# opencv/opencv_contrib

Hardware: AMD Instinct MI355X
Metric: frame-pairs/sec dense TV-L1 flow @1080p (higher is better)
Workload: dtype f32; 1 GPU; DualTVL1 dense flow, 1920x1080 CV_32FC1, 64 pairs/GPU/step (BASELINE configs[1]; 64 pairs/GPU = the per-GPU share of ~; warps=5, nscales=5, semantics=CPU_REF, math=fast, lanes=2

## Files before the change

opencv_contrib_amd/csrc/mi_common.cpp:

```cpp
#include "mi_common.h"
#include <vector>
#include <cstdlib>
#include <cstring>
#include <cstdio>
#include <mutex>

namespace mi {
static Tuning g_tuning;
static std::once_flag g_tuning_once;
static int env_int(const char *name, int dflt)
{
    const char *e = getenv(name);
    return e && *e ? atoi(e) : dflt;
}
#ifdef MIFLOW_EXPERIMENTS
#define EXP_INT(name, dflt) env_int(name, dflt)
#define EXP_ENV(name) getenv(name)
#else
#define EXP_INT(name, dflt) (dflt)
#define EXP_ENV(name) ((const char *)nullptr)
#endif
#ifndef MIFLOW_EXPERIMENTS
extern "C" char **environ;
static void warn_unread_switches()
{
    static const char *const known[] = {"MIFLOW_BF_W", "MIFLOW_CACHE_GB", "MIFLOW_CACHE_TOTAL_GB", "MIFLOW_FB_FUSE", "MIFLOW_FB_GROUP_MB", "MIFLOW_FB_NARROW",
                                        "MIFLOW_FB_PAIR", "MIFLOW_LANES", "MIFLOW_MULTI_RCCL", "MIFLOW_SURF_NMS0", "MIFLOW_SURF_POLY", "MIFLOW_SURF_STAGE_S",
                                        "MIFLOW_TB_HIST", "MIFLOW_TB_VERBOSE", "MIFLOW_TILE_MAXPX"};
    static const char *const foreign[] = {"MIFLOW_LIB", "MIFLOW_BENCH_", "MIFLOW_SWEEP_", "MIFLOW_BUILD_", "MIFLOW_EXTRA_", "MIFLOW_SLP_"};
    if (!environ) return;
    for (char **e = environ; *e; ++e) {
        if (strncmp(*e, "MIFLOW_", 7) != 0) continue;
        const char *eq = strchr(*e, '=');
        const size_t n = eq ? (size_t)(eq - *e) : strlen(*e);
        bool ok = false;
        for (const char *k : known) ok = ok || (strlen(k) == n && strncmp(k, *e, n) == 0);
        for (const char *k : foreign) ok = ok || strncmp(k, *e, strlen(k)) == 0;
        if (!ok) fprintf(stderr, "miflow: %.*s is not read by this library (tuning experiments exist in the -DMIFLOW_EXPERIMENTS build only); ignored\n", (int)n, *e);
    }
}
#endif
const Tuning &tuning()
{
    std::call_once(g_tuning_once, [] {
        Tuning &t = g_tuning;
#ifndef MIFLOW_EXPERIMENTS
        warn_unread_switches();
#endif
        t.x_skip = EXP_INT("MIFLOW_X_SKIP", 0);
        t.warp_tile = EXP_INT("MIFLOW_WARP_TILE", 32);
        if (t.warp_tile != 64 && t.warp_tile != 32 && t.warp_tile != 16) t.warp_tile = 32;
        t.warp_lds = EXP_INT("MIFLOW_WARP_LDS", 0);
        t.warp_fast = EXP_INT("MIFLOW_WARP_FAST", -1);
        t.warp_np = EXP_INT("MIFLOW_WARP_NP", 2);
        if (t.warp_np != 1 && t.warp_np != 4) t.warp_np = 2;
        t.tb_swz = EXP_INT("MIFLOW_TB_SWZ", 1);
        t.tb_p16 = EXP_INT("MIFLOW_TB_P16", 0);
        t.tb_nograd = EXP_INT("MIFLOW_TB_NOGRAD", 1);
        t.tb_skip_p = EXP_INT("MIFLOW_TB_SKIP_P", 1);
        t.tb_hist = env_int("MIFLOW_TB_HIST", 1);
        t.fb_poll = EXP_INT("MIFLOW_FB_POLL", 1);
        t.fb_ahead = EXP_INT("MIFLOW_FB_AHEAD", 1);
        t.tb_fw = EXP_INT("MIFLOW_TB_FW", 0);
        t.tb_jw = EXP_INT("MIFLOW_TB_JW", 2);
        if (t.tb_jw < 0 || t.tb_jw > 4) t.tb_jw = 2;
        t.tb_jw_spec = EXP_INT("MIFLOW_TB_JW_SPEC", 1);
        t.tb_ppl = t.tb_wps = t.tb_pf = -1;
        if (const char *v = EXP_ENV("MIFLOW_TB_VARIANT")) (void)sscanf(v, "%d,%d,%d", &t.tb_ppl, &t.tb_wps, &t.tb_pf);
        t.tb_force = EXP_ENV("MIFLOW_TB_FORCE") != nullptr;
        t.tb_plan_wps = EXP_INT("MIFLOW_TB_WPS", 0);
        t.tb_rows = EXP_INT("MIFLOW_TB_ROWS", 0);
        t.tb_rows_equal = EXP_INT("MIFLOW_TB_ROWS_EQUAL", 0);
        t.tb_il = EXP_INT("MIFLOW_TB_IL", 1);
        t.tb_verbose = getenv("MIFLOW_TB_VERBOSE") != nullptr;
        {
            const char *e = getenv("MIFLOW_TILE_MAXPX");
            t.tile_maxpx = e && *e ? atoll(e) : 2300000;
        }
        t.tile_variant = EXP_INT("MIFLOW_TILE_VARIANT", -1);
        t.tile_small_wgs = EXP_INT("MIFLOW_TILE_SMALL_WGS", 1024);
        t.tile_swz = EXP_INT("MIFLOW_TILE_SWZ", 1);
        t.warp_swz = EXP_INT("MIFLOW_WARP_SWZ", 1);
        t.tile_fb_block = EXP_INT("MIFLOW_TILE_FB_BLOCK", 10);
        t.tile_fb_model = EXP_INT("MIFLOW_TILE_FB_MODEL", 7);
        t.tile_spec = EXP_INT("MIFLOW_TILE_SPEC", 1);
        t.lanes = env_int("MIFLOW_LANES", 0);
        t.spec = EXP_INT("MIFLOW_SPEC", 1);
        t.exact_tb = EXP_INT("MIFLOW_EXACT_TB", 1);
        t.fb_tiled = EXP_INT("MIFLOW_FB_TILED", 1);
        t.sbm_wt = EXP_INT("MIFLOW_SBM_WT", 1);
        t.sbm_swz = EXP_INT("MIFLOW_SBM_SWZ", 1);
        t.sbm_texfuse = EXP_INT("MIFLOW_SBM_TEXFUSE", 1);
        t.fb_rows = EXP_INT("MIFLOW_FB_ROWS", 4) == 8 ? 8 : 4;
        t.fb_group_mb = env_int("MIFLOW_FB_GROUP_MB", 240);
        t.fb_fuse = env_int("MIFLOW_FB_FUSE", -1);
        t.fb_pair = env_int("MIFLOW_FB_PAIR", -1);
        t.fb_narrow = env_int("MIFLOW_FB_NARROW", -1);
        t.fb_swz = EXP_INT("MIFLOW_FB_SWZ", 1);
        t.fb_group_streams = EXP_INT("MIFLOW_FB_GROUP_STREAMS", 2);
        t.fb_poly_tiled = EXP_INT("MIFLOW_FB_POLY_TILED", 1);
        t.fb_direct = EXP_INT("MIFLOW_FB_DIRECT", 1);
        t.fb_blur_tiled = EXP_INT("MIFLOW_FB_BLUR_TILED", 1);
    });
    return g_tuning;
}

namespace {
struct BigBlock { void *p; size_t cap; int dev; hipEvent_t ready; };
std::mutex g_big_mu;
std::vector<BigBlock> g_big;
const size_t kBigMaxBlocks = 4;
size_t big_max_bytes()
{
    static const size_t v = [] {
        const char *e = getenv("MIFLOW_CACHE_GB");
        const long long gb = e && *e ? atoll(e) : 24;
        return (size_t)(gb < 0 ? 0 : gb) << 30;
    }();
    return v;
}
size_t big_max_bytes_total()
{
    static const size_t v = [] {
        const char *e = getenv("MIFLOW_CACHE_TOTAL_GB");
        if (e && *e) { const long long gb = atoll(e); return (size_t)(gb < 0 ? 0 : gb) << 30; }
        return 4 * big_max_bytes();
    }();
    return v;
}
}

int big_alloc(void **p, size_t bytes, size_t *capacity)
{
    int dev = 0;
    MI_HIP_TRY(hipGetDevice(&dev));
    {
        hipEvent_t ready = nullptr;
        bool hit = false;
        {
            std::lock_guard<std::mutex> lk(g_big_mu);
            int best = -1;
            for (size_t i = 0; i < g_big.size(); ++i)
                if (g_big[i].dev == dev && g_big[i].cap >= bytes && g_big[i].cap <= bytes + bytes / 2 + (64u << 20) &&
                    (best < 0 || g_big[i].cap < g_big[best].cap))
                    best = (int)i;
            if (best >= 0) {
                *p = g_big[best].p; *capacity = g_big[best].cap; ready = g_big[best].ready;
                g_big.erase(g_big.begin() + best);
                hit = true;
            }
        }
        if (hit) {
            if (ready) {
                const hipError_t we = hipEventSynchronize(ready);
                (void)hipEventDestroy(ready);
                if (we != hipSuccess) {
                    (void)hipGetLastError();
                    if (hipDeviceSynchronize() != hipSuccess) { (void)hipGetLastError(); (void)hipFree(*p); *p = nullptr; hit = false; }
                }
            }
            if (hit) return MI_OK;
        }
    }
    hipError_t e = hipMalloc(p, bytes);
    if (e != hipSuccess) {
        big_trim();
        e = hipMalloc(p, bytes);
    }
    if (e != hipSuccess) { set_error("hipMalloc of %zu bytes failed: %s", bytes, hipGetErrorString(e)); return MI_ERR_OOM; }
    *capacity = bytes;
    return MI_OK;
}

void big_free(void *p, size_t capacity, hipEvent_t ready, bool busy)
{
    if (!p) { if (ready) (void)hipEventDestroy(ready); return; }
    int dev = 0;
    void *drop = nullptr;
    if (hipGetDevice(&dev) == hipSuccess) {
        hipPointerAttribute_t at;
        const int cur = dev;
        if (hipPointerGetAttributes(&at, p) == hipSuccess) dev = at.device;
        if (dev != cur) (void)hipSetDevice(dev);
        bool idle = true;
        if (!ready && busy) idle = hipDeviceSynchronize() == hipSuccess;
        if (dev != cur) (void)hipSetDevice(cur);
        std::lock_guard<std::mutex> lk(g_big_mu);
        size_t total = capacity, all = capacity, blocks = 0;
        for (const BigBlock &b : g_big) {
            all += b.cap;
            if (b.dev == dev) { total += b.cap; ++blocks; }
        }
        if (idle && blocks < kBigMaxBlocks && total <= big_max_bytes() && all <= big_max_bytes_total()) {
            g_big.push_back({p, capacity, dev, ready});
            return;
        }
        if (ready) { (void)hipEventSynchronize(ready); (void)hipEventDestroy(ready); }
        drop = p;
    } else {
        if (ready) (void)hipEventDestroy(ready);
        drop = p;
    }
    const hipError_t fe = hipFree(drop);
    if (fe != hipSuccess) set_error("hipFree of a %zu-byte arena failed: %s", capacity, hipGetErrorString(fe));
}

void big_trim()
{
    std::vector<BigBlock> all;
    {
        std::lock_guard<std::mutex> lk(g_big_mu);
        all.swap(g_big);
    }
    int cur = 0;
    const bool have = hipGetDevice(&cur) == hipSuccess;
    for (const BigBlock &b : all) {
        if (b.ready) { (void)hipEventSynchronize(b.ready); (void)hipEventDestroy(b.ready); }
        (void)hipFree(b.p);
    }
    if (have) (void)hipSetDevice(cur);
}

int device_simds()
{
    static std::mutex mu;
    static int cache[64];
    int dev = 0;
    if (hipGetDevice(&dev) != hipSuccess || dev < 0 || dev >= 64) return 1024;
    std::lock_guard<std::mutex> lk(mu);
    if (!cache[dev]) {
        int cus = 0;
        if (hipDeviceGetAttribute(&cus, hipDeviceAttributeMultiprocessorCount, dev) != hipSuccess || cus <= 0) cus = 256;
        cache[dev] = 4 * cus;
    }
    return cache[dev];
}

static thread_local char g_err[512] = "";
void set_error(const char *fmt, ...)
{
    va_list ap;
    va_start(ap, fmt);
    vsnprintf(g_err, sizeof(g_err), fmt, ap);
    va_end(ap);
}

int require_device()
{
    int n = 0;
    MI_REQUIRE(hipGetDeviceCount(&n) == hipSuccess && n > 0, MI_ERR_NO_DEVICE,
               "no HIP device available: the miflow product path has no CPU fallback");
    return MI_OK;
}
}

extern "C" {

const char *mi_last_error(void) { return mi::g_err; }
#ifdef MIFLOW_EXPERIMENTS
const char *mi_version(void) { return "miflow 0.1 (gfx950) +experiments"; }
#else
const char *mi_version(void) { return "miflow 0.1 (gfx950)"; }
#endif

int mi_device_count(void)
{
    int n = 0;
    if (hipGetDeviceCount(&n) != hipSuccess) return 0;
    return n;
}
int mi_set_device(int device) { MI_HIP_TRY(hipSetDevice(device)); return MI_OK; }
int mi_release_cached_memory(void) { mi::big_trim(); return MI_OK; }
int mi_get_device(int *device) { MI_REQUIRE(device, MI_ERR_BAD_ARG, "null device"); MI_HIP_TRY(hipGetDevice(device)); return MI_OK; }

int mi_malloc(void **dptr, size_t bytes)
{
    MI_REQUIRE(dptr, MI_ERR_BAD_ARG, "null dptr");
    MI_HIP_TRY(hipMalloc(dptr, bytes ? bytes : 1));
    return MI_OK;
}
int mi_malloc_pitch(void **dptr, size_t *step, size_t width_bytes, int rows)
{
    MI_REQUIRE(dptr && step && rows >= 0, MI_ERR_BAD_ARG, "bad mi_malloc_pitch arguments");
    const size_t st = rows > 1 ? (width_bytes + 255) / 256 * 256 : width_bytes;
    MI_HIP_TRY(hipMalloc(dptr, st * (size_t)(rows ? rows : 1) + 16));
    *step = st;
    return MI_OK;
}
int mi_free(void *dptr) { MI_HIP_TRY(hipFree(dptr)); return MI_OK; }
int mi_memcpy_h2d(void *dst, size_t dstep, const void *src, size_t sstep, size_t width_bytes, int rows, void *stream)
{
    MI_HIP_TRY(hipMemcpy2DAsync(dst, dstep, src, sstep, width_bytes, (size_t)rows, hipMemcpyHostToDevice, (hipStream_t)stream));
    return MI_OK;
}
int mi_memcpy_d2h(void *dst, size_t dstep, const void *src, size_t sstep, size_t width_bytes, int rows, void *stream)
{
    MI_HIP_TRY(hipMemcpy2DAsync(dst, dstep, src, sstep, width_bytes, (size_t)rows, hipMemcpyDeviceToHost, (hipStream_t)stream));
    return MI_OK;
}
int mi_memset(void *dst, size_t dstep, int value, size_t width_bytes, int rows, void *stream)
{
    MI_HIP_TRY(hipMemset2DAsync(dst, dstep, value, width_bytes, (size_t)rows, (hipStream_t)stream));
    return MI_OK;
}
int mi_stream_create(void **stream)
{
    MI_REQUIRE(stream, MI_ERR_BAD_ARG, "null stream");
    hipStream_t s;
    MI_HIP_TRY(hipStreamCreateWithFlags(&s, hipStreamNonBlocking));
    *stream = (void *)s;
    return MI_OK;
}
int mi_stream_destroy(void *stream) { MI_HIP_TRY(hipStreamDestroy((hipStream_t)stream)); return MI_OK; }
int mi_stream_synchronize(void *stream) { MI_HIP_TRY(hipStreamSynchronize((hipStream_t)stream)); return MI_OK; }

}
```

opencv_contrib_amd/csrc/mi_common.h:

```cpp
#pragma once
#include <vector>
#include <hip/hip_runtime.h>
#include <cstdarg>
#include <cstdio>
#include <cstring>
#include "miflow/c_api.h"
#include "mi_buf.h"

namespace mi {

#define MI_HIP_TRY(expr)                                                                  \
    do {                                                                                  \
        hipError_t _e = (expr);                                                           \
        if (_e != hipSuccess) {                                                           \
            mi::set_error("%s failed: %s (%s:%d)", #expr, hipGetErrorString(_e), __FILE__, __LINE__); \
            return _e == hipErrorOutOfMemory ? MI_ERR_OOM : MI_ERR_HIP;                   \
        }                                                                                 \
    } while (0)

#define MI_REQUIRE(cond, code, ...)        \
    do {                                   \
        if (!(cond)) {                     \
            mi::set_error(__VA_ARGS__);    \
            return (code);                 \
        }                                  \
    } while (0)

#define MI_TRY(expr) do { if (const int _rc = (expr)) return _rc; } while (0)

struct Tuning {
    int x_skip;
    int warp_tile;
    int warp_lds;
    int warp_fast;
    int warp_np;
    int tb_swz;
    int tb_p16;
    int tb_nograd;
    int tb_hist;
    int fb_poll;
    int fb_ahead;
    int tb_skip_p;
    int tb_fw;
    int tb_jw;
    int tb_jw_spec;
    int tb_ppl, tb_wps, tb_pf;
    int tb_force;
    int tb_plan_wps;
    int tb_rows;
    int tb_rows_equal;
    int tb_il;
    int tb_verbose;
    long long tile_maxpx;
    int tile_spec;
    int tile_variant;
    int tile_fb_block;
    int tile_fb_model;
    int tile_swz, warp_swz;
    int tile_small_wgs;
    int lanes;
    int exact_tb;
    int spec;
    int sbm_texfuse;
    int sbm_swz;
    int sbm_wt;
    int fb_rows, fb_swz;
    int fb_group_mb;
    int fb_fuse;
    int fb_pair;
    int fb_narrow;
    int fb_group_streams;
    int fb_poly_tiled;
    int fb_direct;
    int fb_blur_tiled;
    int fb_tiled;
};
const Tuning &tuning();
#ifdef MIFLOW_EXPERIMENTS
#define MI_EXP_ENV(name) getenv(name)
#else
#define MI_EXP_ENV(name) ((const char *)nullptr)
#endif

int require_device();

struct DevAlloc {
    static int alloc(void **p, size_t bytes) { MI_HIP_TRY(hipMalloc(p, bytes)); return MI_OK; }
    static void free(void *p) { (void)hipFree(p); }
};
template <unsigned Flags>
struct PinnedAlloc {
    static int alloc(void **p, size_t bytes) { MI_HIP_TRY(hipHostMalloc(p, bytes, Flags)); return MI_OK; }
    static void free(void *p) { (void)hipHostFree(p); }
};
template <class T> using DevBuf = GrowBuf<T, DevAlloc>;
template <class T, unsigned Flags> using PinnedBuf = GrowBuf<T, PinnedAlloc<Flags>>;

struct DevTmp {
    std::vector<void *> bufs;
    DevTmp() = default;
    DevTmp(const DevTmp &) = delete;
    DevTmp &operator=(const DevTmp &) = delete;
    ~DevTmp() { for (void *p : bufs) DevAlloc::free(p); }
    template <class T>
    int alloc(T **out, size_t n)
    {
        void *p = nullptr;
        *out = nullptr;
        if (const int rc = DevAlloc::alloc(&p, sizeof(T) * n)) return rc;
        bufs.push_back(p);
        *out = (T *)p;
        return MI_OK;
    }
};

int big_alloc(void **p, size_t bytes, size_t *capacity);
void big_free(void *p, size_t capacity, hipEvent_t ready = nullptr, bool busy = true);
void big_trim();
int device_simds();

static inline int div_up(int a, int b) { return (a + b - 1) / b; }
static inline int align_up(int a, int b) { return div_up(a, b) * b; }

struct PlaneF {
    float *p;
    int ld;
};

}
```

opencv_contrib_amd/csrc/tvl1_api.cpp:

```cpp
#include "tvl1_dev.h"
#include "mi_selftest.h"
#include <cfloat>
#include <algorithm>
#include <cmath>
#include <vector>
#include <chrono>
#include <sched.h>
#include <time.h>

using namespace mi;
using namespace mi::tvl1;

namespace {

constexpr double kFeedbackWaitLimitUs = 30e6;

struct LevelBuf {
    Geo g;
    float *I0 = nullptr, *I1 = nullptr;
    float *u[2][3] = {{nullptr, nullptr, nullptr}, {nullptr, nullptr, nullptr}};
};

struct SlotInfo { int scale, warp; };

}

struct Lane {
    int capW = 0, capH = 0, capB = 0, capScales = 0;
    double capStep = 0;
    bool capGamma = false, capMedian = false;
    float *arena = nullptr;
    size_t arena_bytes = 0;
    std::vector<LevelBuf> L;
    float *scr[6] = {};
    float *pbuf[2][6] = {};
    DevBuf<PtrTab> tab;
    std::vector<PtrTab> tab_host;
    DevBuf<int2> S;
    DevBuf<unsigned long long> E;
    DevBuf<double> Pd;
    DevBuf<int4> X;
    long long Q = 0;
    int ctlB = 0;
    DevBuf<int> H;
    unsigned long long H_sig = 0;
    int H_par = 0;
    std::vector<SlotInfo> slots;
    PinnedBuf<int2, hipHostMallocDefault> fb_host;
    hipEvent_t fb_ev = nullptr;
    PinnedBuf<int, hipHostMallocCoherent | hipHostMallocMapped> fb_flag;
    int fb_seq = 0;
    std::vector<int> fb_hist;
    unsigned long long fb_hist_sig = 0;
    std::vector<hipEvent_t> ev_pool;
    struct Region { int e0, e1; long long launches; double bytes; int kind; int level; };
    std::vector<Region> regions;
    hipStream_t stream = nullptr;
    hipEvent_t done = nullptr;
    hipEvent_t idle_ev = nullptr;
    bool idle_valid = false;
    bool used = false;
};

struct mi_tvl1 {
    mi_tvl1_params P;
    int device = 0;
    DevBuf<float> cubic_tab;
    static const int kMaxLanes = 4;
    Lane lane[kMaxLanes];
    hipEvent_t fork = nullptr;
    int last_nscales = 0, last_batch = 0, last_lanes = 1;
    int last_first[kMaxLanes + 1] = {};
    bool last_check = false;
    bool profiling = false;
};

void mi_tvl1_default_params(mi_tvl1_params *p)
{
    if (!p) return;
    p->tau = 0.25; p->lambda = 0.15; p->theta = 0.3; p->epsilon = 0.01; p->scale_step = 0.8; p->gamma = 0.0;
    p->nscales = 5; p->warps = 5; p->iterations = 300; p->use_initial_flow = 0;
    p->inner_iterations = 1; p->median_filtering = 1;
    p->semantics = MI_SEM_CPU_REF; p->exact_math = 0; p->time_block = 0; p->lanes = 0; p->stop_slack = 0; p->host_feedback = 0;
}

static const long long kMaxSlots = 4000000;

static int validate_params(const mi_tvl1_params *p)
{
    MI_REQUIRE(p, MI_ERR_BAD_ARG, "null params");
    MI_REQUIRE(p->nscales > 0 && p->nscales <= 32, MI_ERR_BAD_ARG, "nscales must be in [1,32] (CV_Assert nscales_ > 0)");
    MI_REQUIRE(p->warps >= 0 && p->warps <= 64, MI_ERR_BAD_ARG, "warps must be in [0,64]");
    MI_REQUIRE(p->iterations >= 0 && p->inner_iterations >= 0, MI_ERR_BAD_ARG, "negative iteration count");
    MI_REQUIRE((long long)p->iterations * p->inner_iterations <= kMaxSlots, MI_ERR_BAD_ARG,
               "iterations x inner_iterations must not exceed %lld", kMaxSlots);
    MI_REQUIRE(p->scale_step > 0 && p->scale_step < 1, MI_ERR_BAD_ARG, "scale_step must be in (0,1)");
    MI_REQUIRE(p->theta != 0, MI_ERR_BAD_ARG, "theta must be non-zero");
    MI_REQUIRE(p->semantics == MI_SEM_CPU_REF || p->semantics == MI_SEM_CUDA_COMPAT, MI_ERR_BAD_ARG, "bad semantics");
    MI_REQUIRE(p->median_filtering <= 1 || p->median_filtering == 3 || p->median_filtering == 5, MI_ERR_BAD_ARG,
               "medianFiltering must be 1 (off), 3 or 5 (cv::medianBlur on CV_32F)");
    MI_REQUIRE(p->lanes >= 0 && p->lanes <= 4, MI_ERR_BAD_ARG, "lanes must be 0 (automatic) or 1..4");
    MI_REQUIRE(p->stop_slack >= 0 && p->stop_slack <= 8, MI_ERR_BAD_ARG, "stop_slack must be in 0..8");
    MI_REQUIRE(p->host_feedback >= -1 && p->host_feedback <= 1, MI_ERR_BAD_ARG, "host_feedback must be -1, 0 or 1");
    return MI_OK;
}

int mi_tvl1_create(const mi_tvl1_params *p, mi_tvl1 **out)
{
    MI_REQUIRE(out, MI_ERR_BAD_ARG, "null out");
    *out = nullptr;
    mi_tvl1_params d;
    if (!p) { mi_tvl1_default_params(&d); p = &d; }
    int rc = validate_params(p);
    if (rc) return rc;
    MI_TRY(require_device());
    mi_tvl1 *h = new mi_tvl1();
    h->P = *p;
    float tab[128];
    host_cubic_table(tab);
    auto upload = [&]() -> int {
        MI_HIP_TRY(hipGetDevice(&h->device));
        MI_TRY(h->cubic_tab.ensure(128));
        MI_HIP_TRY(hipMemcpy(h->cubic_tab.p, tab, sizeof(tab), hipMemcpyHostToDevice));
        return MI_OK;
    };
    if (const int rc = upload()) { mi_tvl1_destroy(h); return rc; }
    *out = h;
    return MI_OK;
}

int mi_tvl1_set_params(mi_tvl1 *h, const mi_tvl1_params *p)
{
    MI_REQUIRE(h, MI_ERR_BAD_ARG, "null handle");
    int rc = validate_params(p);
    if (rc) return rc;
    h->P = *p;
    return MI_OK;
}

int mi_tvl1_get_params(const mi_tvl1 *h, mi_tvl1_params *p)
{
    MI_REQUIRE(h && p, MI_ERR_BAD_ARG, "null argument");
    *p = h->P;
    return MI_OK;
}

static void free_arena(Lane &ln)
{
    if (ln.arena) {
        big_free(ln.arena, ln.arena_bytes, ln.idle_valid ? ln.idle_ev : nullptr, ln.used);
        if (ln.idle_valid) ln.idle_ev = nullptr;
    }
    ln.idle_valid = false;
    ln.used = false;
    ln.arena = nullptr;
    ln.L.clear();
}

int mi_tvl1_query_plan(int width, int height, int pairs_per_lane, int iterations_per_launch, int *kernel, int *rows_per_band)
{
    MI_REQUIRE(kernel && rows_per_band, MI_ERR_BAD_ARG, "null output");
    MI_REQUIRE(width > 0 && height > 0 && pairs_per_lane > 0 && iterations_per_launch > 0, MI_ERR_BAD_ARG, "bad plan query");
    int dev = 0;
    if (hipGetDevice(&dev) != hipSuccess) { set_error("no HIP device"); return MI_ERR_NO_DEVICE; }
    const Geo g{width, height, (width + 63) / 64 * 64, (long long)((width + 63) / 64 * 64) * height, pairs_per_lane};
    const TbKernel k = tb_kernel(TbUse::Fixed, iterations_per_launch, g, false, false, tv_knobs(), TbOverride{});
    if (!k.tile && !k.row) { set_error("unsupported time block %d", iterations_per_launch); return MI_ERR_BAD_ARG; }
    *kernel = k.tile ? 1 : 0;
    *rows_per_band = k.tile ? tile_owned_rows() : plan_band_rows(*k.row, g);
    return MI_OK;
}

int mi_tvl1_set_profiling(mi_tvl1 *h, int enable)
{
    MI_REQUIRE(h, MI_ERR_BAD_ARG, "null handle");
    h->profiling = enable != 0;
    return MI_OK;
}

int mi_tvl1_get_profile(mi_tvl1 *h, double *ms_total, long long *launches, double *algo_bytes)
{
    return mi_tvl1_get_profile_kind(h, 0, ms_total, launches, algo_bytes);
}

int mi_tvl1_get_profile_kind(mi_tvl1 *h, int kind, double *ms_total, long long *launches, double *algo_bytes)
{
    return mi_tvl1_get_profile_level(h, kind, -1, ms_total, launches, algo_bytes);
}

int mi_tvl1_get_profile_level(mi_tvl1 *h, int kind, int level, double *ms_total, long long *launches, double *algo_bytes)
{
    MI_REQUIRE(h && ms_total && launches && algo_bytes, MI_ERR_BAD_ARG, "null argument");
    MI_REQUIRE(kind == 0 || kind == 1, MI_ERR_BAD_ARG, "kind must be 0 (iteration launches) or 1 (warp launches)");
    *ms_total = 0; *launches = 0; *algo_bytes = 0;
    for (int li = 0; li < h->last_lanes; ++li) {
        Lane &ln = h->lane[li];
        for (const auto &r : ln.regions) {
            if (r.kind != kind || (level >= 0 && r.level != level)) continue;
            MI_HIP_TRY(hipEventSynchronize(ln.ev_pool[r.e1]));
            float ms = 0.f;
            MI_HIP_TRY(hipEventElapsedTime(&ms, ln.ev_pool[r.e0], ln.ev_pool[r.e1]));
            *ms_total += ms; *launches += r.launches; *algo_bytes += r.bytes;
        }
    }
    return MI_OK;
}

void mi_tvl1_destroy(mi_tvl1 *h)
{
    if (!h) return;
    for (Lane &ln : h->lane) {
        for (hipEvent_t e : ln.ev_pool) (void)hipEventDestroy(e);
        free_arena(ln);
        if (ln.idle_ev) { (void)hipEventDestroy(ln.idle_ev); ln.idle_ev = nullptr; }
        if (ln.done) (void)hipEventDestroy(ln.done);
        if (ln.fb_ev) (void)hipEventDestroy(ln.fb_ev);
        if (ln.stream) (void)hipStreamDestroy(ln.stream);
    }
    if (h->fork) (void)hipEventDestroy(h->fork);
    delete h;
}

static int ensure_arena(const mi_tvl1_params &P, Lane &ln, const TvPlan &pl, int W, int H, int B)
{
    const bool gam = P.gamma != 0.0, med = pl.median != 0;
    if (!(ln.arena && ln.capW == W && ln.capH == H && ln.capB >= B && ln.capScales == P.nscales && ln.capStep == P.scale_step &&
          ln.capGamma == gam && ln.capMedian == med)) {
        free_arena(ln);
        void *blk = nullptr;
        if (const int rc = big_alloc(&blk, pl.arena.total * sizeof(float), &ln.arena_bytes)) return rc;
        ln.arena = (float *)blk;
        const auto at = [&](size_t o) { return o == kNoPlane ? nullptr : ln.arena + o; };
        ln.L.resize(pl.geo.size());
        for (size_t l = 0; l < pl.geo.size(); ++l) {
            ln.L[l].I0 = at(pl.arena.lv[l][0]); ln.L[l].I1 = at(pl.arena.lv[l][1]);
            for (int k = 0; k < 6; ++k) ln.L[l].u[k / 3][k % 3] = at(pl.arena.lv[l][2 + k]);
        }
        for (int k = 0; k < 6; ++k) ln.scr[k] = at(pl.arena.scr[k]);
        for (int k = 0; k < 12; ++k) ln.pbuf[k / 6][k % 6] = at(pl.arena.p[k]);
        ln.capGamma = gam; ln.capMedian = med; ln.capW = W; ln.capH = H; ln.capB = B; ln.capScales = P.nscales; ln.capStep = P.scale_step;
    }
    for (size_t l = 0; l < pl.geo.size(); ++l) ln.L[l].g = pl.geo[l];
    return MI_OK;
}

static int check_pair(const mi_mat *I0, const mi_mat *I1, const mi_mat *flow, const mi_mat *I0ref)
{
    MI_REQUIRE(I0 && I1 && flow, MI_ERR_BAD_ARG, "null matrix");
    MI_REQUIRE(I0->data && I1->data && flow->data, MI_ERR_BAD_ARG, "null data pointer");
    MI_REQUIRE(I0->type == MI_8UC1 || I0->type == MI_32FC1, MI_ERR_BAD_TYPE, "I0 must be CV_8UC1 or CV_32FC1");
    MI_REQUIRE(I0->rows == I1->rows && I0->cols == I1->cols, MI_ERR_BAD_SIZE, "I0.size() != I1.size()");
    MI_REQUIRE(I0->type == I1->type, MI_ERR_BAD_TYPE, "I0.type() != I1.type()");
    MI_REQUIRE(flow->type == MI_32FC2, MI_ERR_BAD_TYPE, "flow must be CV_32FC2");
    MI_REQUIRE(flow->rows == I0->rows && flow->cols == I0->cols, MI_ERR_BAD_SIZE, "flow.size() != I0.size()");
    MI_REQUIRE(I0->rows >= 3 && I0->cols >= 3, MI_ERR_BAD_SIZE, "image must be at least 3x3");
    MI_REQUIRE((long long)((I0->cols + 63) / 64 * 64) * I0->rows * 4 < (1LL << 32), MI_ERR_BAD_SIZE,
               "image too large: a float plane of it must stay below 4 GiB");
    const size_t es = I0->type == MI_8UC1 ? 1 : 4;
    MI_REQUIRE(I0->step >= (size_t)I0->cols * es && I1->step >= (size_t)I1->cols * es, MI_ERR_BAD_ARG, "step < cols*elemSize");
    MI_REQUIRE(flow->step >= (size_t)flow->cols * 8, MI_ERR_BAD_ARG, "flow step < cols*8");
    if (es == 4) MI_REQUIRE(I0->step % 4 == 0 && I1->step % 4 == 0 && ((uintptr_t)I0->data % 4) == 0 && ((uintptr_t)I1->data % 4) == 0,
                            MI_ERR_BAD_ARG, "float images must be 4-byte aligned");
    MI_REQUIRE(flow->step % 8 == 0 && ((uintptr_t)flow->data % 8) == 0, MI_ERR_BAD_ARG, "flow must be 8-byte aligned");
    MI_REQUIRE(I0->rows == I0ref->rows && I0->cols == I0ref->cols && I0->type == I0ref->type, MI_ERR_BAD_SIZE,
               "all pairs of a batch must share size and type");
    return MI_OK;
}

const TvKnobs &mi::tvl1::tv_knobs()
{
    static const TvKnobs k = [] {
        const Tuning &t = tuning();
        TvKnobs v{};
        v.tile_maxpx = t.tile_maxpx; v.tile_spec = t.tile_spec; v.tile_variant = t.tile_variant; v.tile_small_wgs = t.tile_small_wgs;
        v.tile_variants = std::min(tile_variants(), (int)(sizeof(v.tile_rows) / sizeof(v.tile_rows[0])));
        for (int i = 0; i < v.tile_variants; ++i) v.tile_rows[i] = tile_shape_rows(i);
        v.tile_fb_block = t.tile_fb_block; v.tile_fb_model = t.tile_fb_model;
        v.tb_force = t.tb_force != 0; v.tb_nograd = t.tb_nograd; v.tb_jw = t.tb_jw; v.tb_jw_spec = t.tb_jw_spec;
        v.tb_ppl = t.tb_ppl; v.tb_wps = t.tb_wps; v.tb_pf = t.tb_pf; v.tb_p16 = t.tb_p16; v.tb_il = t.tb_il;
        v.tb_fw = t.tb_fw; v.tb_skip_p = t.tb_skip_p; v.tb_hist = t.tb_hist; v.spec = t.spec; v.exact_tb = t.exact_tb;
        v.fb_poll = t.fb_poll; v.fb_ahead = t.fb_ahead; v.warp_fast = t.warp_fast; v.warp_lds = t.warp_lds; v.x_skip = t.x_skip;
        return v;
    }();
    return k;
}

static int ensure_buffers(const TvPlan &pl, Lane &ln, int B, const mi_mat *I0s, const mi_mat *I1s, mi_mat *flows, hipStream_t st)
{
    int rc;
    if ((rc = ln.tab.ensure(B))) return rc;
    ln.tab_host.resize(B);
    for (int i = 0; i < B; ++i)
        ln.tab_host[i] = PtrTab{I0s[i].data, I1s[i].data, flows[i].data, (long long)I0s[i].step, (long long)I1s[i].step, (long long)flows[i].step};
    MI_HIP_TRY(hipMemcpyAsync(ln.tab.p, ln.tab_host.data(), sizeof(PtrTab) * B, hipMemcpyHostToDevice, st));
    if (pl.check) {
        MI_REQUIRE(pl.Q <= kMaxSlots, MI_ERR_BAD_ARG, "scales x warps x iterations = %lld control slots exceed the limit of %lld", pl.Q, kMaxSlots);
        if (ln.Q < pl.Q || ln.ctlB < B) {
            const size_t n = (size_t)pl.Q * B;
            if ((rc = ln.S.ensure(n)) || (rc = ln.E.ensure(n)) || (rc = ln.Pd.ensure(n)) || (rc = ln.X.ensure(n))) return rc;
            ln.Q = pl.Q; ln.ctlB = B;
        }
        MI_HIP_TRY(hipMemsetAsync(ln.E.p, 0, sizeof(unsigned long long) * (size_t)ln.Q * B, st));
        MI_HIP_TRY(hipMemsetAsync(ln.S.p, 0, sizeof(int2) * (size_t)ln.Q * B, st));
    }
    if (pl.hist) {
        const int nw = (int)pl.warp[0].size();
        const size_t h_n = (size_t)pl.used * nw * B;
        if (ln.H.n < 2 * h_n) ln.H_sig = 0;
        if ((rc = ln.H.ensure(2 * h_n))) return rc;
        if (ln.H_sig != pl.hist_sig) {
            MI_HIP_TRY(hipMemsetAsync(ln.H.p, 0, sizeof(int) * ln.H.n, st));
            ln.H_sig = pl.hist_sig;
        }
        if (ln.fb_hist_sig != pl.hist_sig || ln.fb_hist.size() != (size_t)pl.used * nw) {
            ln.fb_hist.assign((size_t)pl.used * nw, 0);
            ln.fb_hist_sig = pl.hist_sig;
        }
        ln.H_par ^= 1;
    }
    if (pl.fb) {
        const bool fresh = ln.fb_flag.n < 2 * (size_t)B;
        if ((rc = ln.fb_host.ensure(2 * (size_t)B)) || (rc = ln.fb_flag.ensure(2 * (size_t)B))) return rc;
        if (fresh) memset(ln.fb_flag.p, 0, sizeof(int) * ln.fb_flag.n);
        if (!ln.fb_ev) MI_HIP_TRY(hipEventCreateWithFlags(&ln.fb_ev, hipEventDisableTiming));
    }
    return MI_OK;
}

namespace {

struct Run {
    mi_tvl1 *h;
    Lane &ln;
    const TvPlan &pl;
    const TvKnobs &K;
    hipStream_t st;
    int B;
    size_t ev_used = 0;
    Ctl ctl;
    IterPlanes planes;
    float *grad = nullptr;
    float l_t, theta, taut;
    int q = 0, q_last = -1, e_next = 0;
    int q_settle_prev = -1, q_settle_scale = -1;
    int fb_prev_warp = 2, fb_prev_scale = 2;
    int cur = 0;
    bool first_of_scale = true;
    bool pre_warped = false;
};

int record(Run &r, int *idx)
{
    if (r.ev_used == r.ln.ev_pool.size()) {
        hipEvent_t e;
        MI_HIP_TRY(hipEventCreate(&e));
        r.ln.ev_pool.push_back(e);
    }
    *idx = (int)r.ev_used++;
    MI_HIP_TRY(hipEventRecord(r.ln.ev_pool[*idx], r.st));
    return MI_OK;
}

int enqueue_pyramid(Run &r, int type)
{
    const mi_tvl1_params &P = r.h->P;
    Lane &ln = r.ln;
    const int ns = r.pl.used, B = r.B;
    int rc = convert(ln.tab.p, type, ln.L[0].I0, ln.L[0].I1, ln.L[0].g, r.st);
    if (rc) return rc;
    if (P.use_initial_flow && (rc = unpack_flow(ln.tab.p, ln.L[0].u[0][0], ln.L[0].u[0][1], ln.L[0].g, r.st))) return rc;
    const float one3[3] = {1.f, 1.f, 1.f};
    for (size_t s = 1; s < ln.L.size(); ++s) {
        const LevelBuf &c = ln.L[s - 1];
        const float *src[3][2] = {{c.I0, nullptr}, {c.I1, nullptr}, {nullptr, nullptr}};
        float *dst[3] = {ln.L[s].I0, ln.L[s].I1, nullptr};
        rc = resize(P.semantics, 2, src, 1, dst, c.g, ln.L[s].g, P.scale_step, P.scale_step, one3, nullptr, 0, r.st);
        if (rc) return rc;
        if ((int)s >= ns) break;
        if (P.use_initial_flow) {
            const float *us[3][2] = {{c.u[0][0], nullptr}, {c.u[0][1], nullptr}, {nullptr, nullptr}};
            float *ud[3] = {ln.L[s].u[0][0], ln.L[s].u[0][1], nullptr};
            const float post[3] = {(float)P.scale_step, (float)P.scale_step, 1.f};
            rc = resize(P.semantics, 2, us, 1, ud, c.g, ln.L[s].g, P.scale_step, P.scale_step, post, nullptr, 0, r.st);
            if (rc) return rc;
        }
    }
    const LevelBuf &Lc = ln.L[ns - 1];
    const size_t bytes = sizeof(float) * (size_t)Lc.g.ps * B;
    if (!P.use_initial_flow) {
        MI_HIP_TRY(hipMemsetAsync(Lc.u[0][0], 0, bytes, r.st));
        MI_HIP_TRY(hipMemsetAsync(Lc.u[0][1], 0, bytes, r.st));
    }
    if (P.gamma != 0.0) MI_HIP_TRY(hipMemsetAsync(Lc.u[0][2], 0, bytes, r.st));
    return MI_OK;
}

int launch_warp(Run &r, const LevelBuf &Lv, bool ahead)
{
    const float *u1v[2] = {Lv.u[0][0], Lv.u[1][0]}, *u2v[2] = {Lv.u[0][1], Lv.u[1][1]};
    Ctl c = r.ctl;
    c.q_prev = r.q_last;
    c.need_done = ahead ? 1 : 0;
    const bool dev_cur = ahead || (r.pl.check && !r.first_of_scale);
    return warp_fused(r.h->P.semantics, r.pl.fast_warp, -1, Lv.I0, Lv.I1, u1v, u2v, nullptr, r.ln.scr[2], r.ln.scr[3],
                      r.grad, r.ln.scr[5], r.h->cubic_tab.p, Lv.g, dev_cur ? &c : nullptr, r.cur, r.st);
}

int run_blocked(Run &r, LevelBuf &Lv, const TvWarp &w, long long *nlaunch)
{
    float *const mu1[2] = {Lv.u[0][0], Lv.u[1][0]}, *const mu2[2] = {Lv.u[0][1], Lv.u[1][1]};
    const int nb = (int)w.blocks.size();
    int rc;
    for (int no = 0; no < w.outer; ++no) {
        if (r.pl.median && (rc = median_flow(r.pl.median, mu1, mu2, r.ln.scr[0], r.ln.scr[1], Lv.g, nullptr, r.cur, r.st))) return rc;
        for (int k = 0; k < nb; ++k) {
            ++*nlaunch;
            if (w.skip_iterations) { r.first_of_scale = false; continue; }
            const bool last_pass = w.skip_p_last && no == w.outer - 1 && k == nb - 1;
            rc = w.fused ? iterate_tb_fused(w.run[k], Lv.I0, Lv.I1, r.h->cubic_tab.p, r.planes, Lv.g, r.l_t, r.theta, r.taut, r.first_of_scale, r.cur,
                                            r.st, last_pass)
                         : iterate_tb(w.run[k], w.blocks[k], r.planes, Lv.g, r.l_t, r.theta, r.taut, r.first_of_scale, r.cur, r.st, last_pass,
                                      last_pass && w.pack_in_pass ? r.ln.tab.p : nullptr);
            if (rc) return rc;
            r.cur ^= 1;
            r.first_of_scale = false;
        }
    }
    return MI_OK;
}

int run_per_iteration(Run &r, LevelBuf &Lv, int s, int wp, long long *nlaunch)
{
    const mi_tvl1_params &P = r.h->P;
    const int mf = r.pl.median;
    float *const mu1[2] = {Lv.u[0][0], Lv.u[1][0]}, *const mu2[2] = {Lv.u[0][1], Lv.u[1][1]};
    int rc;
    for (int it = 0; it < r.pl.iters; ++it) {
        ++*nlaunch;
        if (mf && it % P.inner_iterations == 0) {
            Ctl mc = r.ctl;
            mc.q_prev = r.q_last; mc.first_of_warp = (it == 0); mc.reset_cur = r.first_of_scale;
            if ((rc = median_flow(mf, mu1, mu2, r.ln.scr[0], r.ln.scr[1], Lv.g, r.pl.check ? &mc : nullptr, r.cur, r.st))) return rc;
        }
        if (r.pl.check) {
            Ctl ic = r.ctl;
            ic.q = r.q; ic.q_prev = r.q_last; ic.first_of_warp = (it == 0); ic.reset_cur = r.first_of_scale; ic.n = it;
            rc = iterate(P.exact_math != 0, r.planes, Lv.g, r.l_t, r.theta, r.taut, r.first_of_scale, &ic, 0, r.st);
            r.ln.slots.push_back({s, wp});
            r.q_last = r.q++;
        } else {
            rc = iterate(P.exact_math != 0, r.planes, Lv.g, r.l_t, r.theta, r.taut, r.first_of_scale, nullptr, r.cur, r.st);
            r.cur ^= 1;
        }
        if (rc) return rc;
        r.first_of_scale = false;
    }
    return MI_OK;
}

struct Feedback { bool all = true, all_before = true; int n_most = 0; };

int poll_feedback(Run &r, int seq, Feedback *f)
{
    const int *flag = r.ln.fb_flag.p;
    for (int b = 0; b < r.B; ++b) {
        int v = 0;
        const auto t_wait0 = std::chrono::steady_clock::now();
        for (long long spin = 0;; ++spin) {
            v = __atomic_load_n(flag + 2 * b, __ATOMIC_ACQUIRE);
            if ((v >> 2) == seq) break;
            if ((spin & 63) != 63) {
#if defined(__x86_64__) || defined(__i386__)
                __builtin_ia32_pause();
#endif
                continue;
            }
            const double waited_us = std::chrono::duration<double, std::micro>(std::chrono::steady_clock::now() - t_wait0).count();
            if (waited_us < 20.0) continue;
            const hipError_t qe = hipStreamQuery(r.st);
            if (qe != hipErrorNotReady) {
                v = __atomic_load_n(flag + 2 * b, __ATOMIC_ACQUIRE);
                if ((v >> 2) == seq) break;
                MI_HIP_TRY(qe);
                MI_REQUIRE(false, MI_ERR_HIP, "host feedback: launch finished without publishing its decision");
            }
            MI_REQUIRE(waited_us < kFeedbackWaitLimitUs, MI_ERR_HIP, "host feedback: no decision from the device within %.0f s", kFeedbackWaitLimitUs * 1e-6);
            if (waited_us < 2000.0) sched_yield();
            else { struct timespec ts_ = {0, 50000}; nanosleep(&ts_, nullptr); }
        }
        f->all_before = f->all_before && (v & 2);
        f->all = f->all && (v & 1);
        f->n_most = std::max(f->n_most, flag[2 * b + 1]);
    }
    return MI_OK;
}

int copy_feedback(Run &r, Feedback *f)
{
    Lane &ln = r.ln;
    MI_HIP_TRY(hipMemcpy2DAsync(ln.fb_host.p, 2 * sizeof(int2), ln.S.p + (r.q_last - 1), sizeof(int2) * (size_t)ln.Q, 2 * sizeof(int2),
                                (size_t)r.B, hipMemcpyDeviceToHost, r.st));
    MI_HIP_TRY(hipEventRecord(ln.fb_ev, r.st));
    MI_HIP_TRY(hipEventSynchronize(ln.fb_ev));
    for (int b = 0; b < r.B; ++b) {
        f->all_before = f->all_before && (ln.fb_host.p[2 * b].y & MI_SLOT_DONE);
        f->all = f->all && (ln.fb_host.p[2 * b + 1].y & MI_SLOT_DONE);
    }
    return MI_OK;
}

int run_spec(Run &r, LevelBuf &Lv, const TvWarp &w, int s, int wp, long long *nlaunch)
{
    const TvPlan &pl = r.pl;
    Lane &ln = r.ln;
    const int nw = (int)pl.warp[s].size();
    int rc, hprev = 0;
    if (pl.fb_poll && pl.hist) {
        int &hc = ln.fb_hist[(size_t)s * nw + wp];
        hprev = hc;
        hc = 0;
    }
    const std::vector<int> plan = spec_blocks(w, Lv.g, hprev, r.K);
    int t_after = 0;
    for (int v : plan) t_after += v;
    SpecK sk;
    memset(&sk, 0, sizeof(sk));
    sk.X = ln.X.p; sk.iters = pl.iters;
    sk.q_hist = wp > 0 ? r.q_settle_prev : r.q_settle_scale;
    spec_hist_fraction(wp, &sk.hist_num, &sk.hist_den);
    sk.slack = r.h->P.stop_slack;
    if (pl.hist) {
        const size_t o = ((size_t)s * nw + wp) * r.B, half = ln.H.n / 2;
        sk.h_in = ln.H.p + (size_t)(ln.H_par ^ 1) * half + o;
        sk.h_out = ln.H.p + (size_t)ln.H_par * half + o;
    }
    if (r.first_of_scale) {
        const size_t n = (size_t)Lv.g.ps * r.B;
        if ((rc = zero_planes4(ln.pbuf[0], n, r.st))) return rc;
        float *const p3[4] = {ln.pbuf[0][4], ln.pbuf[0][5], ln.pbuf[0][4], ln.pbuf[0][5]};
        if (r.h->P.gamma != 0.0 && (rc = zero_planes4(p3, n, r.st))) return rc;
    }
    int e_prev = 0;
    int fb_next = pl.fb ? spec_first_poll(plan, hprev, wp > 0 ? r.fb_prev_warp : r.fb_prev_scale) : -1;
    int fb_done_at = (int)plan.size();
    for (size_t k = 0; k <= plan.size(); ++k) {
        const bool last = k == plan.size();
        const int T = last ? plan.back() : plan[k];
        if (!last) t_after -= T;
        Ctl a = r.ctl;
        a.q = r.q; a.q_prev = r.q_last; a.first_of_warp = (k == 0); a.reset_cur = (k == 0 && r.first_of_scale); a.n = 0;
        sk.e0_prev = e_prev; sk.final_launch = last ? 1 : 0; sk.t_after = t_after;
        if (pl.fb_poll) {
            ln.fb_seq = (ln.fb_seq + 1) & 0x0fffffff;
            sk.fb_flag = ln.fb_flag.p; sk.fb_seq = ln.fb_seq;
        }
        MI_REQUIRE((long long)r.e_next + T <= ln.Q && r.q < ln.Q, MI_ERR_BAD_ARG,
                   "speculative steps: error-sum slot %d + %d or launch slot %d beyond the %lld slots sized for this calc", r.e_next, T, r.q, ln.Q);
        const TbKernel kern = tb_kernel(TbUse::Spec, T, Lv.g, r.h->P.gamma != 0.0, w.nograd, r.K);
        if ((rc = iterate_tb_spec(kern, T, r.planes, Lv.g, r.l_t, r.theta, r.taut, a, sk, r.e_next, r.st))) return rc;
        ln.slots.push_back({s, wp});
        r.q_last = r.q++;
        ++*nlaunch;
        e_prev = r.e_next;
        if (!last) r.e_next += T;
        if (!pl.fb || last || (int)k != fb_next) continue;
        const bool ahead = pl.fb_poll && r.K.fb_ahead != 0 && r.K.x_skip == 0 && !r.h->profiling && wp + 1 < nw;
        if (ahead && (rc = launch_warp(r, Lv, true))) return rc;
        Feedback f;
        if ((rc = pl.fb_poll ? poll_feedback(r, ln.fb_seq, &f) : copy_feedback(r, &f))) return rc;
        if (f.all) {
            r.pre_warped = ahead;
            if (pl.fb_poll && pl.hist) ln.fb_hist[(size_t)s * nw + wp] = f.n_most;
            fb_done_at = f.all_before ? (int)k - 1 : (int)k;
            break;
        }
        fb_next = (int)k + 2;
    }
    if (pl.fb) {
        r.fb_prev_warp = fb_done_at;
        if (wp == 0) r.fb_prev_scale = fb_done_at;
    }
    r.q_settle_prev = r.q_last;
    if (wp == 0) r.q_settle_scale = r.q_last;
    r.first_of_scale = false;
    return MI_OK;
}

int run_warp(Run &r, LevelBuf &Lv, int s, int wp)
{
    const TvWarp &w = r.pl.warp[s][wp];
    const Geo &g = Lv.g;
    const bool prof = r.h->profiling;
    int rc, w0 = -1, w1 = -1, e0 = -1, e1 = -1;
    r.planes.g = r.grad = w.nograd ? nullptr : r.ln.scr[4];
    if (prof && (rc = record(r, &w0))) return rc;
    if (r.pre_warped) r.pre_warped = false;
    else if (w.warp_launch && (rc = launch_warp(r, Lv, false))) return rc;
    if (prof && !w.fused) {
        if ((rc = record(r, &w1))) return rc;
        r.ln.regions.push_back({w0, w1, 1, 44.0 * g.w * g.h * r.B, 1, s});
    }
    if (prof && r.pl.iters > 0 && (rc = record(r, &e0))) return rc;
    long long nlaunch = 0;
    switch (w.form) {
    case TvForm::Blocked:
    case TvForm::ExactBlocked: rc = run_blocked(r, Lv, w, &nlaunch); break;
    case TvForm::Spec: rc = run_spec(r, Lv, w, s, wp, &nlaunch); break;
    case TvForm::PerIter: rc = run_per_iteration(r, Lv, s, wp, &nlaunch); break;
    }
    if (rc) return rc;
    if (e0 >= 0) {
        if ((rc = record(r, &e1))) return rc;
        r.ln.regions.push_back({e0, e1, nlaunch, 64.0 * g.w * g.h * r.B * r.pl.iters, 0, s});
    }
    return MI_OK;
}

int zoom_or_pack(Run &r, int s)
{
    const mi_tvl1_params &P = r.h->P;
    const LevelBuf &Lv = r.ln.L[s];
    Ctl ec = r.ctl;
    ec.q_prev = r.q_last;
    const Ctl *dev = r.pl.check && !r.first_of_scale ? &ec : nullptr;
    if (s == 0) {
        if (!r.pl.warp[0].empty() && r.pl.warp[0].back().pack_in_pass) return MI_OK;
        const float *u1v[2] = {Lv.u[0][0], Lv.u[1][0]}, *u2v[2] = {Lv.u[0][1], Lv.u[1][1]};
        return pack_flow(r.ln.tab.p, u1v, u2v, Lv.g, dev, r.cur, r.st);
    }
    const LevelBuf &Lf = r.ln.L[s - 1];
    const bool gam = P.gamma != 0.0;
    const float *us[3][2] = {{Lv.u[0][0], Lv.u[1][0]}, {Lv.u[0][1], Lv.u[1][1]}, {gam ? Lv.u[0][2] : nullptr, gam ? Lv.u[1][2] : nullptr}};
    float *ud[3] = {Lf.u[0][0], Lf.u[0][1], gam ? Lf.u[0][2] : nullptr};
    const float post[3] = {(float)(1.0 / P.scale_step), (float)(1.0 / P.scale_step), 1.f};
    return resize(P.semantics, gam ? 3 : 2, us, 2, ud, Lv.g, Lf.g, (double)Lf.g.w / Lv.g.w, (double)Lf.g.h / Lv.g.h, post, dev, r.cur, r.st);
}

}

static int lane_calc(mi_tvl1 *h, Lane &ln, int n, const mi_mat *I0s, const mi_mat *I1s, mi_mat *flows, hipStream_t st, int *ns_out)
{
    struct Mark {
        Lane &l; hipStream_t s;
        ~Mark()
        {
            if (!l.arena) return;
            l.used = true; l.idle_valid = false;
            hipStreamCaptureStatus cs = hipStreamCaptureStatusNone;
            if (hipStreamIsCapturing(s, &cs) != hipSuccess || cs != hipStreamCaptureStatusNone) { (void)hipGetLastError(); return; }
            if (!l.idle_ev && hipEventCreateWithFlags(&l.idle_ev, hipEventDisableTiming) != hipSuccess) { l.idle_ev = nullptr; (void)hipGetLastError(); return; }
            if (hipEventRecord(l.idle_ev, s) == hipSuccess) l.idle_valid = true; else (void)hipGetLastError();
        }
    } mark{ln, st};
    const mi_tvl1_params &P = h->P;
    hipStreamCaptureStatus cap_st = hipStreamCaptureStatusNone;
    const bool capturing = hipStreamIsCapturing(st, &cap_st) == hipSuccess && cap_st != hipStreamCaptureStatusNone;
    const TvPlan pl = tv_make_plan(TvShape{I0s[0].cols, I0s[0].rows, n, I0s[0].type, P, h->last_lanes, capturing}, tv_knobs());
    int rc = ensure_arena(P, ln, pl, I0s[0].cols, I0s[0].rows, n);
    if (rc || (rc = ensure_buffers(pl, ln, n, I0s, I1s, flows, st))) return rc;
    if (!pl.warp.empty() && !pl.warp[0].empty() && pl.warp[0].back().pack_in_pass)
        for (int i = 0; i < n; ++i) MI_REQUIRE(flows[i].step < (1ll << 31), MI_ERR_BAD_ARG, "flow matrix pitch of %lld bytes", (long long)flows[i].step);
    *ns_out = pl.used;
    ln.slots.clear();
    ln.regions.clear();

    Run r{h, ln, pl, tv_knobs(), st, n};
    memset(&r.ctl, 0, sizeof(r.ctl));
    r.ctl.S = ln.S.p; r.ctl.E = ln.E.p; r.ctl.Q = (int)ln.Q; r.ctl.P = ln.Pd.p;
    r.ctl.sched = P.semantics == MI_SEM_CUDA_COMPAT ? 1 : 0;
    r.l_t = (float)(P.lambda * P.theta); r.taut = (float)(P.tau / P.theta); r.theta = (float)P.theta;
    if ((rc = enqueue_pyramid(r, I0s[0].type))) return rc;
    for (int s = pl.used - 1; s >= 0; --s) {
        LevelBuf &Lv = ln.L[s];
        IterPlanes &ip = r.planes;
        ip.ix = ln.scr[2]; ip.iy = ln.scr[3]; ip.rc = ln.scr[5]; ip.gamma = (float)P.gamma;
        for (int k = 0; k < 2; ++k) { for (int j = 0; j < 3; ++j) ip.u[k][j] = Lv.u[k][j]; for (int j = 0; j < 6; ++j) ip.p[k][j] = ln.pbuf[k][j]; }
        ip.err_u3 = P.semantics == MI_SEM_CPU_REF ? 1 : 0;
        r.cur = 0; r.first_of_scale = true; r.pre_warped = false;
        const double se = P.epsilon * P.epsilon * (double)(Lv.g.w * Lv.g.h);
        r.ctl.thr = P.semantics == MI_SEM_CPU_REF ? (double)(float)se : se;
        for (int wp = 0; wp < P.warps; ++wp)
            if ((rc = run_warp(r, Lv, s, wp))) return rc;
        if ((rc = zoom_or_pack(r, s))) return rc;
    }
    return MI_OK;
}

int mi_tvl1_calc_batch(mi_tvl1 *h, int n, const mi_mat *I0s, const mi_mat *I1s, mi_mat *flows, void *stream_)
{
    MI_REQUIRE(h, MI_ERR_BAD_ARG, "null handle");
    MI_REQUIRE(n > 0 && I0s && I1s && flows, MI_ERR_BAD_ARG, "empty batch");
    hipStream_t st = (hipStream_t)stream_;
    for (int i = 0; i < n; ++i) {
        int rc = check_pair(&I0s[i], &I1s[i], &flows[i], &I0s[0]);
        if (rc) return rc;
    }
    int lanes = h->P.lanes > 0 ? h->P.lanes : (tuning().lanes > 0 ? tuning().lanes : (n >= 4 ? 2 : 1));
    if (lanes > mi_tvl1::kMaxLanes) lanes = mi_tvl1::kMaxLanes;
    if (lanes > n) lanes = n;
    int ns = 0;
    h->last_check = h->P.epsilon > 0.0 && h->P.iterations * h->P.inner_iterations > 0;
    h->last_batch = n; h->last_lanes = lanes;
    for (int i = 0; i <= lanes; ++i) h->last_first[i] = (int)((long long)n * i / lanes);
    if (lanes == 1) {
        int rc = lane_calc(h, h->lane[0], n, I0s, I1s, flows, st, &ns);
        if (rc) return rc;
    } else {
        if (!h->fork) MI_HIP_TRY(hipEventCreateWithFlags(&h->fork, hipEventDisableTiming));
        for (int li = 1; li < lanes; ++li) {
            Lane &ln = h->lane[li];
            if (!ln.stream) MI_HIP_TRY(hipStreamCreateWithFlags(&ln.stream, hipStreamNonBlocking));
            if (!ln.done) MI_HIP_TRY(hipEventCreateWithFlags(&ln.done, hipEventDisableTiming));
        }
        MI_HIP_TRY(hipEventRecord(h->fork, st));
        int rc_first = MI_OK;
        auto note = [&](hipError_t e) {
            if (e != hipSuccess && !rc_first) { set_error("HIP error in the lane fork / join: %s", hipGetErrorString(e)); rc_first = MI_ERR_HIP; }
            return e == hipSuccess;
        };
        for (int li = lanes - 1; li >= 0; --li) {
            Lane &ln = h->lane[li];
            const int off = h->last_first[li], cnt = h->last_first[li + 1] - off;
            hipStream_t ls = li > 0 ? ln.stream : st;
            const bool forked = li == 0 || note(hipStreamWaitEvent(ln.stream, h->fork, 0));
            if (forked && !rc_first) {
                const int rc = lane_calc(h, ln, cnt, I0s + off, I1s + off, flows + off, ls, &ns);
                if (rc && !rc_first) rc_first = rc;
            }
        }
        for (int li = 1; li < lanes; ++li) {
            Lane &ln = h->lane[li];
            if (!(note(hipEventRecord(ln.done, ln.stream)) && note(hipStreamWaitEvent(st, ln.done, 0)))) (void)hipStreamSynchronize(ln.stream);
        }
        if (rc_first) return rc_first;
    }
    h->last_nscales = ns;
    if (ns < h->P.nscales) h->P.nscales = ns;
    return MI_OK;
}

int mi_tvl1_calc(mi_tvl1 *h, const mi_mat *I0, const mi_mat *I1, mi_mat *flow, void *stream)
{
    return mi_tvl1_calc_batch(h, 1, I0, I1, flow, stream);
}

static int read_slots(mi_tvl1 *h, int pair, hipStream_t stream, const Lane **lane, std::vector<int2> *S, std::vector<int4> *X,
                      int cap_launches = -1)
{
    int li = 0;
    while (li + 1 < h->last_lanes && pair >= h->last_first[li + 1]) ++li;
    const Lane &ln = h->lane[li];
    const size_t off = (size_t)(pair - h->last_first[li]) * ln.Q;
    const int nq = (int)ln.slots.size();
    MI_REQUIRE(cap_launches < 0 || nq <= cap_launches, MI_ERR_BAD_ARG, "capacity too small");
    *lane = &ln;
    S->resize(nq);
    MI_HIP_TRY(hipStreamSynchronize(stream));
    MI_HIP_TRY(hipMemcpy(S->data(), ln.S.p + off, sizeof(int2) * nq, hipMemcpyDeviceToHost));
    if (X) {
        X->resize(nq);
        if (ln.X.p) MI_HIP_TRY(hipMemcpy(X->data(), ln.X.p + off, sizeof(int4) * nq, hipMemcpyDeviceToHost));
    }
    return MI_OK;
}

int mi_tvl1_last_iterations(mi_tvl1 *h, int pair, int *nscales_used, int *iters, int cap, void *stream)
{
    MI_REQUIRE(h && iters && nscales_used, MI_ERR_BAD_ARG, "null argument");
    MI_REQUIRE(pair >= 0 && pair < h->last_batch, MI_ERR_BAD_ARG, "pair index out of range");
    const int ns = h->last_nscales, nw = h->P.warps;
    MI_REQUIRE(cap >= ns * nw, MI_ERR_BAD_ARG, "iters capacity too small");
    *nscales_used = ns;
    for (int i = 0; i < ns * nw; ++i) iters[i] = 0;
    if (!h->last_check) {
        for (int i = 0; i < ns * nw; ++i) iters[i] = h->P.iterations * h->P.inner_iterations;
        return MI_OK;
    }
    const Lane *ln = nullptr;
    std::vector<int2> S;
    if (const int rc = read_slots(h, pair, (hipStream_t)stream, &ln, &S, nullptr)) return rc;
    for (size_t i = 0; i < S.size(); ++i) {
        const int k = (S[i].y >> 8) & 0xff;
        iters[ln->slots[i].scale * nw + ln->slots[i].warp] += k ? k : (S[i].y & 1);
    }
    return MI_OK;
}

int miflow_selftest_tvl1_slots(mi_tvl1 *h, int pair, int *out_host, int cap_launches, void *stream)
{
    MI_REQUIRE(h && out_host, MI_ERR_BAD_ARG, "null argument");
    MI_REQUIRE(pair >= 0 && pair < h->last_batch, MI_ERR_BAD_ARG, "pair out of range");
    if (!h->last_check) return 0;
    const Lane *ln = nullptr;
    std::vector<int2> S;
    std::vector<int4> X;
    if (const int rc = read_slots(h, pair, (hipStream_t)stream, &ln, &S, &X, cap_launches)) return rc;
    const int nq = (int)S.size();
    for (int i = 0; i < nq; ++i) {
        int *o = out_host + 8 * i;
        o[0] = ln->slots[i].scale; o[1] = ln->slots[i].warp; o[2] = S[i].x; o[3] = S[i].y;
        o[4] = X[i].x; o[5] = X[i].y; o[6] = X[i].z; o[7] = X[i].w;
    }
    return nq;
}
```

opencv_contrib_amd/csrc/tvl1_dev.h:

```cpp
#pragma once
#include "mi_common.h"
#include "tvl1_plan.h"

namespace mi {
namespace tvl1 {

const TvKnobs &tv_knobs();

struct Ctl {
    int2 *S;
    unsigned long long *E;
    int Q;
    int q;
    int q_prev;
    int first_of_warp;
    int reset_cur;
    double thr;
    double *P;
    int sched;
    int n;
    int need_done;
};

#define MI_SLOT_FLIP 1
#define MI_SLOT_CHECKED 2
#define MI_SLOT_DONE 4
#define MI_SLOT_ITERS(y) (((y) >> 8) & 0xff)

struct PtrTab {
    const void *a, *b;
    void *out;
    long long step_a, step_b, step_out;
};

struct IterPlanes {
    const float *ix, *iy, *g, *rc;
    float *u[2][3];
    float *p[2][6];
    float gamma;
    int err_u3;
};

int convert(const PtrTab *tab_dev, int type, float *I0, float *I1, const Geo &g, hipStream_t s);
int zero_planes4(float *const p[4], size_t n, hipStream_t s);
int unpack_flow(const PtrTab *tab_dev, float *u1, float *u2, const Geo &g, hipStream_t s);
int pack_flow(const PtrTab *tab_dev, const float *u1[2], const float *u2[2], const Geo &g,
              const Ctl *ctl, int cur_host, hipStream_t s);
int resize(int semantics, int nplanes, const float *const src[3][2], int src_sets, float *const dst[3],
           const Geo &gs, const Geo &gd, double inv_scale_x, double inv_scale_y,
           const float post_scale[3], const Ctl *ctl, int cur_host, hipStream_t s);
int gradient(const float *src, float *dx, float *dy, const Geo &g, hipStream_t s);
int median_flow(int ksize, float *const u1[2], float *const u2[2], float *tmp1, float *tmp2, const Geo &g, const Ctl *ctl, int cur_host,
                hipStream_t s);
int pack3(const float *a, const float *b, const float *c, float *pk, const Geo &g, hipStream_t s);
int warp(int semantics, const float *I0, const float *pk, const float *u1[2], const float *u2[2], float *I1w,
         float *I1wx, float *I1wy, float *grad, float *rho, const float *cubic_tab_dev, const Geo &g, const Ctl *ctl,
         int cur_host, hipStream_t s);
int warp_fused(int semantics, bool fast, int lds, const float *I0, const float *I1, const float *u1[2], const float *u2[2], float *I1w, float *I1wx,
               float *I1wy, float *grad, float *rho, const float *cubic_tab_dev, const Geo &g, const Ctl *ctl, int cur_host,
               hipStream_t s);
int iterate(bool exact, const IterPlanes &pl, const Geo &g, float l_t, float theta, float taut,
            bool p_zero, const Ctl *ctl, int cur_host, hipStream_t s);

int iterate_tb(const TbKernel &k, int T, const IterPlanes &pl, const Geo &g, float l_t, float theta, float taut, bool p_zero, int cur,
               hipStream_t s, bool skip_p_out = false, const PtrTab *out_tab = nullptr);
int iterate_tb_fused(const TbKernel &k, const float *I0, const float *I1, const float *cubic_tab_dev, const IterPlanes &pl, const Geo &g,
                     float l_t, float theta, float taut, bool p_zero, int cur, hipStream_t s, bool skip_p_out);
int iterate_tile(int variant, int nit, const IterPlanes &pl, const Geo &g, float l_t, float theta, float taut, bool p_zero, int cur,
                 hipStream_t s);
int tile_owned_rows();
int tile_shape_rows(int variant);
int plan_band_rows(const TbRow &row, const Geo &g);
int tile_variants();
struct SpecK {
    int4 *X;
    int e0_prev;
    int final_launch;
    int iters;
    int t_after;
    int q_hist;
    int hist_num, hist_den;
    int slack;
    const int *h_in;
    int *h_out;
    int *fb_flag;
    int fb_seq;
};

int iterate_tile_spec(int T, const IterPlanes &pl, const Geo &g, float l_t, float theta, float taut, const Ctl &ctl, const SpecK &sk, int e0,
                      hipStream_t s, int variant = -1);
int iterate_tb_spec(const TbKernel &k, int T, const IterPlanes &pl, const Geo &g, float l_t, float theta, float taut, const Ctl &ctl,
                    const SpecK &sk, int e0, hipStream_t s);
int dbg_lane_shift(int *out_dev, hipStream_t s);
int tb_jw_fault(int *fault_host);

void host_cubic_table(float tab[128]);

}
}
```

opencv_contrib_amd/csrc/tvl1_kernels.hip:

```cpp
#include "tvl1_dev.h"
#include "resize_dev.h"
#include "tvl1_warp_dev.h"
#include "tvl1_tb_dev.h"
#include <cfloat>
#include <cstdlib>
#include <climits>

namespace mi {
namespace tvl1 {

__device__ __forceinline__ float4 ld4(const float *p, long long off, bool ok)
{
    return ok ? *reinterpret_cast<const float4 *>(p + off) : make_float4(0.f, 0.f, 0.f, 0.f);
}
__device__ __forceinline__ void st4(float *p, long long off, bool ok, const float v[4])
{
    if (ok) *reinterpret_cast<float4 *>(p + off) = make_float4(v[0], v[1], v[2], v[3]);
}
#define UNPACK4(dst, v) { dst[0] = v.x; dst[1] = v.y; dst[2] = v.z; dst[3] = v.w; }
__device__ __forceinline__ float lane_prev(float v) { return __shfl_up(v, 1); }
__device__ __forceinline__ float lane_next(float v) { return __shfl_down(v, 1); }


__global__ __launch_bounds__(256) void k_convert(const PtrTab *tab, int type, float *I0, float *I1, Geo g)
{
    const int x = blockIdx.x * 64 + (threadIdx.x & 63);
    const int y = blockIdx.y * 4 + (threadIdx.x >> 6);
    const int b = blockIdx.z;
    if (x >= g.w || y >= g.h) return;
    const PtrTab t = tab[b];
    const long long o = (long long)b * g.ps + (long long)y * g.ld + x;
    if (type == MI_8UC1) {
        I0[o] = (float)((const unsigned char *)t.a)[(long long)y * t.step_a + x];
        I1[o] = (float)((const unsigned char *)t.b)[(long long)y * t.step_b + x];
    } else {
        I0[o] = ((const float *)((const char *)t.a + (long long)y * t.step_a))[x] * 255.0f;
        I1[o] = ((const float *)((const char *)t.b + (long long)y * t.step_b))[x] * 255.0f;
    }
}

__global__ __launch_bounds__(256) void k_unpack_flow(const PtrTab *tab, float *u1, float *u2, Geo g)
{
    const int x = blockIdx.x * 64 + (threadIdx.x & 63);
    const int y = blockIdx.y * 4 + (threadIdx.x >> 6);
    const int b = blockIdx.z;
    if (x >= g.w || y >= g.h) return;
    const PtrTab t = tab[b];
    const float2 f = ((const float2 *)((const char *)t.out + (long long)y * t.step_out))[x];
    const long long o = (long long)b * g.ps + (long long)y * g.ld + x;
    u1[o] = f.x;
    u2[o] = f.y;
}

__global__ __launch_bounds__(256) void k_pack_flow(const PtrTab *tab, const float *u1a, const float *u1b,
                                                   const float *u2a, const float *u2b, Geo g, CtlK ctl, int cur_host)
{
    const int x = blockIdx.x * 64 + (threadIdx.x & 63);
    const int y = blockIdx.y * 4 + (threadIdx.x >> 6);
    const int b = blockIdx.z;
    if (x >= g.w || y >= g.h) return;
    const int cur = resolve_cur_k(ctl, b, cur_host);
    const float *u1 = cur ? u1b : u1a, *u2 = cur ? u2b : u2a;
    const PtrTab t = tab[b];
    const long long o = (long long)b * g.ps + (long long)y * g.ld + x;
    ((float2 *)((char *)t.out + (long long)y * t.step_out))[x] = make_float2(u1[o], u2[o]);
}

__device__ __forceinline__ bool resolve_active_k(const CtlK &c, int b, int cur_host, int &cur)
{
    if (!c.S) { cur = cur_host; return true; }
    if (c.q_prev < 0) { cur = 0; return true; }
    const long long sp = (long long)b * c.Q + c.q_prev;
    const int2 s = c.S[sp];
    cur = c.reset_cur ? 0 : (s.x ^ (s.y & 1));
    if (c.first_of_warp) return true;
    const double e = (double)c.E[sp] * (1.0 / ERR_FIX_SCALE);
    return (s.y & 1) && (!(s.y & 2) || e > c.thr);
}

struct MedArgs { float *u[2][2]; float *tmp[2]; Geo g; };

template <int KS>
__global__ __launch_bounds__(256) void k_median(MedArgs A, CtlK ctl, int cur_host)
{
    constexpr int N = KS * KS, R = KS / 2;
    const int x = blockIdx.x * 64 + (threadIdx.x & 63);
    const int y = blockIdx.y * 4 + (threadIdx.x >> 6);
    const int b = blockIdx.z >> 1, c = blockIdx.z & 1;
    const int W = A.g.w, H = A.g.h, ld = A.g.ld;
    int cur;
    if (!resolve_active_k(ctl, b, cur_host, cur)) return;
    if (x >= W || y >= H) return;
    const float *S = A.u[cur][c] + (long long)b * A.g.ps;
    float v[N];
#pragma unroll
    for (int j = -R; j <= R; ++j)
#pragma unroll
        for (int i = -R; i <= R; ++i)
            v[(j + R) * KS + i + R] = S[(long long)min(max(y + j, 0), H - 1) * ld + min(max(x + i, 0), W - 1)];
#pragma unroll
    for (int i = 0; i <= N / 2; ++i)
#pragma unroll
        for (int j = i + 1; j < N; ++j) {
            const float lo = fminf(v[i], v[j]), hi = fmaxf(v[i], v[j]);
            v[i] = lo; v[j] = hi;
        }
    A.tmp[c][(long long)b * A.g.ps + (long long)y * ld + x] = v[N / 2];
}

__global__ __launch_bounds__(256) void k_median_copy(MedArgs A, CtlK ctl, int cur_host)
{
    const int x = blockIdx.x * 64 + (threadIdx.x & 63);
    const int y = blockIdx.y * 4 + (threadIdx.x >> 6);
    const int b = blockIdx.z >> 1, c = blockIdx.z & 1;
    int cur;
    if (!resolve_active_k(ctl, b, cur_host, cur)) return;
    if (x >= A.g.w || y >= A.g.h) return;
    const long long o = (long long)b * A.g.ps + (long long)y * A.g.ld + x;
    A.u[cur][c][o] = A.tmp[c][o];
}

struct ResizeArgs {
    const float *src[3][2];
    float *dst[3];
    float post[3];
    int nsets, nplanes;
    Geo gs, gd;
    double scale_x, scale_y;
};

#define RSZ_ROWS 8
template <int SEM, int PX, int ROWS>
__global__ __launch_bounds__(256) void k_resize(ResizeArgs A, CtlK ctl, int cur_host)
{
    const int dx = (blockIdx.x * 64 + (threadIdx.x & 63)) * PX;
    const int dy0 = (blockIdx.y * 4 + (threadIdx.x >> 6)) * ROWS;
    const int pl = blockIdx.z % A.nplanes, b = blockIdx.z / A.nplanes;
    if (dx >= A.gd.w || dy0 >= A.gd.h) return;
    const int cur = A.nsets == 2 ? resolve_cur_k(ctl, b, cur_host) : 0;
    const float *S = A.src[pl][cur] + (long long)b * A.gs.ps;
    const int sw = A.gs.w, sh = A.gs.h, ld = A.gs.ld;
    const float ps = A.post[pl];
    RszX X[PX];
#pragma unroll
    for (int j = 0; j < PX; ++j) X[j] = resize_xside<SEM>(min(dx + j, A.gd.w - 1), sw, A.scale_x);
    float *D = A.dst[pl] + (long long)b * A.gd.ps + dx;
#pragma unroll
    for (int r = 0; r < ROWS; ++r) {
        const int dy = dy0 + r;
        if (dy >= A.gd.h) break;
        const RszX Y = resize_yside<SEM>(dy, sh, A.scale_y);
        const float *R0 = S + (long long)Y.i0 * ld, *R1 = S + (long long)Y.i1 * ld;
        float o[PX];
#pragma unroll
        for (int j = 0; j < PX; ++j) {
            o[j] = resize_combine<SEM>(R0, R1, X[j], Y);
            if (ps != 1.0f) o[j] = o[j] * ps;
        }
        if (PX == 4) *reinterpret_cast<float4 *>(D + (long long)dy * A.gd.ld) = make_float4(o[0], o[1], o[2], o[3]);
        else D[(long long)dy * A.gd.ld] = o[0];
    }
}

__global__ __launch_bounds__(256) void k_gradient(const float *src, float *dxp, float *dyp, Geo g)
{
    const int x = blockIdx.x * 64 + (threadIdx.x & 63);
    const int y = blockIdx.y * 4 + (threadIdx.x >> 6);
    const int b = blockIdx.z;
    if (x >= g.w || y >= g.h) return;
    const float *S = src + (long long)b * g.ps;
    const long long r = (long long)y * g.ld;
    const float l = S[r + max(x - 1, 0)], rr = S[r + min(x + 1, g.w - 1)];
    const float u = S[(long long)max(y - 1, 0) * g.ld + x], d = S[(long long)min(y + 1, g.h - 1) * g.ld + x];
    const long long o = (long long)b * g.ps + r + x;
    dxp[o] = 0.5f * (rr - l);
    dyp[o] = 0.5f * (d - u);
}

__global__ __launch_bounds__(256) void k_pack3(const float *a, const float *b_, const float *c, float4 *pk, Geo g)
{
    const int x = blockIdx.x * 64 + (threadIdx.x & 63);
    const int y = blockIdx.y * 4 + (threadIdx.x >> 6);
    const int b = blockIdx.z;
    if (x >= g.w || y >= g.h) return;
    const long long o = (long long)b * g.ps + (long long)y * g.ld + x;
    pk[o] = make_float4(a[o], b_[o], c[o], 0.f);
}

struct WarpArgs {
    const float *I0;
    const float4 *pk;
    const float *u1[2], *u2[2];
    float *I1w, *I1wx, *I1wy, *grad, *rho;
    const float *tab;
    Geo g;
};

__device__ __forceinline__ float bicubic_coeff_cuda(float x_)
{
    const float x = fabsf(x_);
    if (x <= 1.0f) return x * x * (1.5f * x - 2.5f) + 1.0f;
    else if (x < 2.0f) return x * (x * (-0.5f * x + 2.5f) - 4.0f) + 2.0f;
    return 0.0f;
}

template <int SEM, int TX = 64>
__global__ __launch_bounds__(256) void k_warp(WarpArgs A, CtlK ctl, int cur_host)
{
    __shared__ float s_tab[128];
    if (SEM == MI_SEM_CPU_REF) {
        if (threadIdx.x < 128) s_tab[threadIdx.x] = A.tab[threadIdx.x];
        __syncthreads();
    }
    constexpr int TY = 64 / TX;
    const int lane_ = threadIdx.x & 63, wave_ = threadIdx.x >> 6;
    const int x = blockIdx.x * TX + (lane_ % TX);
    const int y = blockIdx.y * (4 * TY) + wave_ * TY + lane_ / TX;
    const int b = blockIdx.z;
    const int W = A.g.w, H = A.g.h, ld = A.g.ld;
    if (x >= W || y >= H) return;
    const int cur = resolve_cur_k(ctl, b, cur_host);
    const long long pb = (long long)b * A.g.ps;
    const long long o = pb + (long long)y * ld + x;
    const float u1v = A.u1[cur][o], u2v = A.u2[cur][o];
    const float4 *P = A.pk + pb;
    float v0, v1, v2;
    if (SEM == MI_SEM_CPU_REF) {
        const float mx = (float)x + u1v, my = (float)y + u2v;
        const int qx = __float2int_rn(mx * 32.0f), qy = __float2int_rn(my * 32.0f);
        const int sx = min(max(qx >> 5, -32768), 32767) - 1;
        const int sy = min(max(qy >> 5, -32768), 32767) - 1;
        const float *wx = s_tab + (qx & 31) * 4, *wy = s_tab + (qy & 31) * 4;
        float w[16];
#pragma unroll
        for (int k1 = 0; k1 < 4; ++k1)
#pragma unroll
            for (int k2 = 0; k2 < 4; ++k2) w[k1 * 4 + k2] = wy[k1] * wx[k2];
        if ((unsigned)sx < (unsigned)max(W - 3, 0) && (unsigned)sy < (unsigned)max(H - 3, 0)) {
            const long long base = (long long)sy * ld + sx;
            float s0, s1, s2;
            {
                const float4 *S = P + base;
                float4 a = S[0], b4 = S[1], c = S[2], d = S[3];
                s0 = a.x * w[0] + b4.x * w[1] + c.x * w[2] + d.x * w[3];
                s1 = a.y * w[0] + b4.y * w[1] + c.y * w[2] + d.y * w[3];
                s2 = a.z * w[0] + b4.z * w[1] + c.z * w[2] + d.z * w[3];
                S += ld; a = S[0]; b4 = S[1]; c = S[2]; d = S[3];
                s0 += a.x * w[4] + b4.x * w[5] + c.x * w[6] + d.x * w[7];
                s1 += a.y * w[4] + b4.y * w[5] + c.y * w[6] + d.y * w[7];
                s2 += a.z * w[4] + b4.z * w[5] + c.z * w[6] + d.z * w[7];
                S += ld; a = S[0]; b4 = S[1]; c = S[2]; d = S[3];
                s0 += a.x * w[8] + b4.x * w[9] + c.x * w[10] + d.x * w[11];
                s1 += a.y * w[8] + b4.y * w[9] + c.y * w[10] + d.y * w[11];
                s2 += a.z * w[8] + b4.z * w[9] + c.z * w[10] + d.z * w[11];
                S += ld; a = S[0]; b4 = S[1]; c = S[2]; d = S[3];
                s0 += a.x * w[12] + b4.x * w[13] + c.x * w[14] + d.x * w[15];
                s1 += a.y * w[12] + b4.y * w[13] + c.y * w[14] + d.y * w[15];
                s2 += a.z * w[12] + b4.z * w[13] + c.z * w[14] + d.z * w[15];
            }
            v0 = s0; v1 = s1; v2 = s2;
        } else if (sx >= W || sx + 4 <= 0 || sy >= H || sy + 4 <= 0) {
            v0 = v1 = v2 = 0.f;
        } else {
            float s0 = 0.f, s1 = 0.f, s2 = 0.f;
            for (int i = 0; i < 4; ++i) {
                const int yi = sy + i;
                if (yi < 0 || yi >= H) continue;
                for (int j = 0; j < 4; ++j) {
                    const int xj = sx + j;
                    if (xj < 0 || xj >= W) continue;
                    const float4 t = P[(long long)yi * ld + xj];
                    s0 += (t.x - 0.f) * w[i * 4 + j];
                    s1 += (t.y - 0.f) * w[i * 4 + j];
                    s2 += (t.z - 0.f) * w[i * 4 + j];
                }
            }
            v0 = s0; v1 = s1; v2 = s2;
        }
    } else {
        const float wxp = (float)x + u1v, wyp = (float)y + u2v;
        const int xmin = (int)ceilf(wxp - 2.0f), xmax = (int)floorf(wxp + 2.0f);
        const int ymin = (int)ceilf(wyp - 2.0f), ymax = (int)floorf(wyp + 2.0f);
        float sum = 0.f, sumx = 0.f, sumy = 0.f, wsum = 0.f;
        for (int cy = ymin; cy <= ymax; ++cy)
            for (int cx = xmin; cx <= xmax; ++cx) {
                const float wgt = bicubic_coeff_cuda(wxp - (float)cx) * bicubic_coeff_cuda(wyp - (float)cy);
                const float4 t = P[(long long)min(max(cy, 0), H - 1) * ld + min(max(cx, 0), W - 1)];
                sum += wgt * t.x;
                sumx += wgt * t.y;
                sumy += wgt * t.z;
                wsum += wgt;
            }
        const float coeff = 1.0f / wsum;
        v0 = sum * coeff; v1 = sumx * coeff; v2 = sumy * coeff;
    }
    if (A.I1w) A.I1w[o] = v0;
    A.I1wx[o] = v1;
    A.I1wy[o] = v2;
    const float Ix2 = v1 * v1, Iy2 = v2 * v2;
    A.grad[o] = Ix2 + Iy2;
    A.rho[o] = (v0 - v1 * u1v - v2 * u2v - A.I0[o]);
}

template <bool EXACT, bool GAMMA = false>
__device__ __forceinline__ void px_update_u(float ix, float iy, float g, float rc, float u1, float u2,
                                            float div1, float div2, float l_t, float theta,
                                            float &u1n, float &u2n, float &err, float gamma = 0.f, float u3 = 0.f,
                                            float div3 = 0.f, float *u3n = nullptr, bool err_u3 = false)
{
    float rho, d1 = 0.f, d2 = 0.f, d3 = 0.f;
    if (EXACT) rho = rc + (ix * u1 + iy * u2);
    else rho = rc + fmaf(ix, u1, iy * u2);
    if (GAMMA) rho = rho + gamma * u3;
    const float ltg = l_t * g;
    if (rho < -ltg) { d1 = l_t * ix; d2 = l_t * iy; if (GAMMA) d3 = l_t * gamma; }
    else if (rho > ltg) { d1 = -l_t * ix; d2 = -l_t * iy; if (GAMMA) d3 = -l_t * gamma; }
    else if (g > FLT_EPSILON) {
        const float fi = EXACT ? (-rho / g) : (-rho * __builtin_amdgcn_rcpf(g));
        d1 = fi * ix; d2 = fi * iy; if (GAMMA) d3 = fi * gamma;
    }
    if (EXACT) {
        const float v1 = u1 + d1, v2 = u2 + d2;
        u1n = v1 + theta * div1;
        u2n = v2 + theta * div2;
    } else {
        u1n = fmaf(theta, div1, u1 + d1);
        u2n = fmaf(theta, div2, u2 + d2);
    }
    const float e1 = u1n - u1, e2 = u2n - u2;
    err = EXACT ? (e1 * e1 + e2 * e2) : fmaf(e1, e1, e2 * e2);
    if (GAMMA) {
        const float v3 = u3 + d3;
        *u3n = v3 + theta * div3;
        const float e3 = *u3n - u3;
        if (err_u3) err = err + e3 * e3;
    }
}

template <bool EXACT>
__device__ __forceinline__ void px_update_p(float ux, float uy, float taut, float &pa, float &pb)
{
    if (EXACT) {
        const float gn = (float)sqrt((double)ux * (double)ux + (double)uy * (double)uy);
        const float ng = 1.0f + taut * gn;
        pa = (pa + taut * ux) / ng;
        pb = (pb + taut * uy) / ng;
    } else {
        const float gn = __builtin_sqrtf(fmaf(ux, ux, uy * uy));
        const float r = __builtin_amdgcn_rcpf(fmaf(taut, gn, 1.0f));
        pa = fmaf(taut, ux, pa) * r;
        pb = fmaf(taut, uy, pb) * r;
    }
}

struct IterArgs {
    IterPlanes pl;
    Geo g;
    float l_t, theta, taut;
    int rows_per_wave;
};

#define STRIP_W 252


struct RowIn {
    float ix[4], iy[4], g[4], rc[4], u1[4], u2[4], p11[4], p12[4], p21[4], p22[4];
    float u3[4], p31[4], p32[4];
};


template <bool PZ, bool GAMMA = false>
__device__ __forceinline__ void load_row(RowIn &r, const IterArgs &A, const float *const u[3], const float *const p[6],
                                         long long off, bool ok)
{
    if (GAMMA) {
        float4 t3 = ld4(u[2], off, ok); UNPACK4(r.u3, t3);
        if (!PZ) {
            t3 = ld4(p[4], off, ok); UNPACK4(r.p31, t3);
            t3 = ld4(p[5], off, ok); UNPACK4(r.p32, t3);
        } else {
#pragma unroll
            for (int j = 0; j < 4; ++j) r.p31[j] = r.p32[j] = 0.f;
        }
    }
    float4 t;
    t = ld4(A.pl.ix, off, ok); UNPACK4(r.ix, t);
    t = ld4(A.pl.iy, off, ok); UNPACK4(r.iy, t);
    t = ld4(A.pl.g, off, ok);  UNPACK4(r.g, t);
    t = ld4(A.pl.rc, off, ok); UNPACK4(r.rc, t);
    t = ld4(u[0], off, ok);    UNPACK4(r.u1, t);
    t = ld4(u[1], off, ok);    UNPACK4(r.u2, t);
    if (!PZ) {
        t = ld4(p[0], off, ok); UNPACK4(r.p11, t);
        t = ld4(p[1], off, ok); UNPACK4(r.p12, t);
        t = ld4(p[2], off, ok); UNPACK4(r.p21, t);
        t = ld4(p[3], off, ok); UNPACK4(r.p22, t);
    } else {
#pragma unroll
        for (int j = 0; j < 4; ++j) r.p11[j] = r.p12[j] = r.p21[j] = r.p22[j] = 0.f;
    }
}

template <bool EXACT, bool GAMMA = false>
__device__ __forceinline__ void row_update_u(const RowIn &r, const float up12[4], const float up22[4],
                                             float l11, float l21, int xb, int y, float l_t, float theta,
                                             float u1n[4], float u2n[4], float e[4], const float up32[4] = nullptr,
                                             float l31 = 0.f, float gamma = 0.f, bool err_u3 = false, float u3n[4] = nullptr)
{
#pragma unroll
    for (int j = 0; j < 4; ++j) {
        const int x = xb + j;
        const float p11l = j ? r.p11[j - 1] : l11;
        const float p21l = j ? r.p21[j - 1] : l21;
        float d1, d2;
        if (y > 0) {
            if (x > 0) {
                d1 = (r.p11[j] - p11l) + (r.p12[j] - up12[j]);
                d2 = (r.p21[j] - p21l) + (r.p22[j] - up22[j]);
            } else {
                d1 = r.p11[j] + r.p12[j] - up12[j];
                d2 = r.p21[j] + r.p22[j] - up22[j];
            }
        } else {
            if (x > 0) {
                d1 = r.p11[j] - p11l + r.p12[j];
                d2 = r.p21[j] - p21l + r.p22[j];
            } else {
                d1 = r.p11[j] + r.p12[j];
                d2 = r.p21[j] + r.p22[j];
            }
        }
        if (GAMMA) {
            const float p31l = j ? r.p31[j - 1] : l31;
            float d3;
            if (y > 0) d3 = x > 0 ? (r.p31[j] - p31l) + (r.p32[j] - up32[j]) : r.p31[j] + r.p32[j] - up32[j];
            else d3 = x > 0 ? r.p31[j] - p31l + r.p32[j] : r.p31[j] + r.p32[j];
            px_update_u<EXACT, true>(r.ix[j], r.iy[j], r.g[j], r.rc[j], r.u1[j], r.u2[j], d1, d2, l_t, theta,
                                     u1n[j], u2n[j], e[j], gamma, r.u3[j], d3, &u3n[j], err_u3);
        } else {
            px_update_u<EXACT>(r.ix[j], r.iy[j], r.g[j], r.rc[j], r.u1[j], r.u2[j], d1, d2, l_t, theta,
                               u1n[j], u2n[j], e[j]);
        }
    }
}

template <bool EXACT, bool PZ, bool CHECK, bool GAMMA = false>
__global__ __launch_bounds__(256) void k_iterate(IterArgs A, CtlK ctl, int cur_host)
{
    const int lane = threadIdx.x & 63, wave = threadIdx.x >> 6;
    const int strip = blockIdx.x, b = blockIdx.z;
    const int band = blockIdx.y * 4 + wave;
    const int W = A.g.w, H = A.g.h, ld = A.g.ld;

    int cur = cur_host;
    bool calc_err = true;
    if (CHECK) {
        int cur_in = 0, active = 1;
        double prev_in = 0.0;
        if (ctl.q_prev >= 0) {
            const long long sp = (long long)b * ctl.Q + ctl.q_prev;
            const int2 s = ctl.S[sp];
            cur_in = ctl.reset_cur ? 0 : (s.x ^ (s.y & 1));
            if (!ctl.first_of_warp) {
                const double e = (double)ctl.E[sp] * (1.0 / ERR_FIX_SCALE);
                const bool checked = (s.y & 2) != 0;
                active = (s.y & 1) && (!checked || e > ctl.thr);
                if (ctl.sched) prev_in = checked ? e : ctl.P[sp] - ctl.thr;
            }
        }
        calc_err = !ctl.sched || ((ctl.n & 1) && prev_in < ctl.thr);
        if (blockIdx.x == 0 && blockIdx.y == 0 && threadIdx.x == 0) {
            ctl.S[(long long)b * ctl.Q + ctl.q] = make_int2(cur_in, active | (calc_err ? 2 : 0));
            if (ctl.sched) ctl.P[(long long)b * ctl.Q + ctl.q] = prev_in;
        }
        if (!active) return;
        cur = cur_in;
    }

    const int y0 = band * A.rows_per_wave;
    if (y0 >= H) return;
    const int y1 = min(y0 + A.rows_per_wave, H);
    const int x0 = strip * STRIP_W;
    const int xb = x0 + lane * 4;
    const bool ok = xb < W;
    const long long pb = (long long)b * A.g.ps;

    const float *uin[3] = {A.pl.u[cur][0] + pb, A.pl.u[cur][1] + pb, GAMMA ? A.pl.u[cur][2] + pb : nullptr};
    const float *pin[6] = {A.pl.p[cur][0] + pb, A.pl.p[cur][1] + pb, A.pl.p[cur][2] + pb, A.pl.p[cur][3] + pb,
                           GAMMA ? A.pl.p[cur][4] + pb : nullptr, GAMMA ? A.pl.p[cur][5] + pb : nullptr};
    float *uout[3] = {A.pl.u[cur ^ 1][0] + pb, A.pl.u[cur ^ 1][1] + pb, GAMMA ? A.pl.u[cur ^ 1][2] + pb : nullptr};
    float *pout[6] = {A.pl.p[cur ^ 1][0] + pb, A.pl.p[cur ^ 1][1] + pb, A.pl.p[cur ^ 1][2] + pb, A.pl.p[cur ^ 1][3] + pb,
                      GAMMA ? A.pl.p[cur ^ 1][4] + pb : nullptr, GAMMA ? A.pl.p[cur ^ 1][5] + pb : nullptr};
    const float gamma = A.pl.gamma;
    const bool err_u3 = A.pl.err_u3 != 0;
    IterArgs B = A;
    B.pl.ix += pb; B.pl.iy += pb; B.pl.g += pb; B.pl.rc += pb;

    float up12[4] = {0, 0, 0, 0}, up22[4] = {0, 0, 0, 0}, up32[4] = {0, 0, 0, 0};
    if (!PZ && y0 > 0) {
        const long long off = (long long)(y0 - 1) * ld + xb;
        float4 t = ld4(pin[1], off, ok); UNPACK4(up12, t);
        t = ld4(pin[3], off, ok); UNPACK4(up22, t);
        if (GAMMA) { t = ld4(pin[5], off, ok); UNPACK4(up32, t); }
    }

    RowIn r;
    float u1c[4], u2c[4], ec[4], u3c[4] = {0, 0, 0, 0};
    {
        const long long off = (long long)y0 * ld + xb;
        load_row<PZ, GAMMA>(r, B, uin, pin, off, ok);
        float l11 = lane_prev(r.p11[3]), l21 = lane_prev(r.p21[3]), l31 = GAMMA ? lane_prev(r.p31[3]) : 0.f;
        if (!PZ && lane == 0 && x0 > 0) {
            l11 = pin[0][(long long)y0 * ld + x0 - 1];
            l21 = pin[2][(long long)y0 * ld + x0 - 1];
            if (GAMMA) l31 = pin[4][(long long)y0 * ld + x0 - 1];
        }
        row_update_u<EXACT, GAMMA>(r, up12, up22, l11, l21, xb, y0, A.l_t, A.theta, u1c, u2c, ec, up32, l31, gamma, err_u3, u3c);
    }
    float errsum = 0.f;
    const bool own = lane < 63;

    for (int y = y0; y < y1; ++y) {
        float p11c[4], p12c[4], p21c[4], p22c[4], p31c[4], p32c[4];
#pragma unroll
        for (int j = 0; j < 4; ++j) { p11c[j] = r.p11[j]; p12c[j] = r.p12[j]; p21c[j] = r.p21[j]; p22c[j] = r.p22[j];
                                      p31c[j] = GAMMA ? r.p31[j] : 0.f; p32c[j] = GAMMA ? r.p32[j] : 0.f; }
        float u1d[4], u2d[4], ed[4], u3d[4] = {0, 0, 0, 0};
        const bool has_next = (y + 1 < H);
        if (has_next) {
            const long long off = (long long)(y + 1) * ld + xb;
            float c12[4], c22[4], c32[4];
#pragma unroll
            for (int j = 0; j < 4; ++j) { c12[j] = r.p12[j]; c22[j] = r.p22[j]; c32[j] = GAMMA ? r.p32[j] : 0.f; }
            load_row<PZ, GAMMA>(r, B, uin, pin, off, ok);
            float l11 = lane_prev(r.p11[3]), l21 = lane_prev(r.p21[3]), l31 = GAMMA ? lane_prev(r.p31[3]) : 0.f;
            if (!PZ && lane == 0 && x0 > 0) {
                l11 = pin[0][(long long)(y + 1) * ld + x0 - 1];
                l21 = pin[2][(long long)(y + 1) * ld + x0 - 1];
                if (GAMMA) l31 = pin[4][(long long)(y + 1) * ld + x0 - 1];
            }
            row_update_u<EXACT, GAMMA>(r, c12, c22, l11, l21, xb, y + 1, A.l_t, A.theta, u1d, u2d, ed, c32, l31, gamma, err_u3, u3d);
        } else {
#pragma unroll
            for (int j = 0; j < 4; ++j) { u1d[j] = u1c[j]; u2d[j] = u2c[j]; u3d[j] = u3c[j]; ed[j] = 0.f; }
        }
        const float r1 = lane_next(u1c[0]), r2 = lane_next(u2c[0]), r3 = GAMMA ? lane_next(u3c[0]) : 0.f;
#pragma unroll
        for (int j = 0; j < 4; ++j) {
            const int x = xb + j;
            const float n1 = j < 3 ? u1c[j + 1] : r1;
            const float n2 = j < 3 ? u2c[j + 1] : r2;
            if (GAMMA) {
                const float n3 = j < 3 ? u3c[j + 1] : r3;
                const float u3x = (x + 1 < W) ? n3 - u3c[j] : 0.f;
                const float u3y = has_next ? u3d[j] - u3c[j] : 0.f;
                px_update_p<EXACT>(u3x, u3y, A.taut, p31c[j], p32c[j]);
            }
            const float u1x = (x + 1 < W) ? n1 - u1c[j] : 0.f;
            const float u2x = (x + 1 < W) ? n2 - u2c[j] : 0.f;
            const float u1y = has_next ? u1d[j] - u1c[j] : 0.f;
            const float u2y = has_next ? u2d[j] - u2c[j] : 0.f;
            px_update_p<EXACT>(u1x, u1y, A.taut, p11c[j], p12c[j]);
            px_update_p<EXACT>(u2x, u2y, A.taut, p21c[j], p22c[j]);
            if (CHECK && own && x < W) errsum += ec[j];
        }
        const long long off = (long long)y * ld + xb;
        const bool st = ok && own;
        st4(uout[0], off, st, u1c);
        st4(uout[1], off, st, u2c);
        st4(pout[0], off, st, p11c);
        st4(pout[1], off, st, p12c);
        st4(pout[2], off, st, p21c);
        st4(pout[3], off, st, p22c);
        if (GAMMA) {
            st4(uout[2], off, st, u3c);
            st4(pout[4], off, st, p31c);
            st4(pout[5], off, st, p32c);
        }
#pragma unroll
        for (int j = 0; j < 4; ++j) { u1c[j] = u1d[j]; u2c[j] = u2d[j]; u3c[j] = u3d[j]; ec[j] = ed[j]; }
    }

    if (CHECK && calc_err) {
        double s = (double)errsum;
#pragma unroll
        for (int o = 32; o > 0; o >>= 1) s += __shfl_xor(s, o);
        if (lane == 0) {
            const unsigned long long f = (unsigned long long)(s * ERR_FIX_SCALE + 0.5);
            atomicAdd(&ctl.E[(long long)b * ctl.Q + ctl.q], f);
        }
    }
}

static inline dim3 grid2d(const Geo &g, int z) { return dim3(div_up(g.w, 64), div_up(g.h, 4), z); }

int convert(const PtrTab *tab, int type, float *I0, float *I1, const Geo &g, hipStream_t s)
{
    hipLaunchKernelGGL(k_convert, grid2d(g, g.batch), dim3(256), 0, s, tab, type, I0, I1, g);
    MI_HIP_TRY(hipGetLastError());
    return MI_OK;
}

__global__ __launch_bounds__(256) void k_zero4(float4 *a, float4 *b, float4 *c, float4 *d, long long n4)
{
    const float4 z = make_float4(0.f, 0.f, 0.f, 0.f);
    for (long long i = (long long)blockIdx.x * 256 + threadIdx.x; i < n4; i += (long long)gridDim.x * 256) {
        a[i] = z; b[i] = z; c[i] = z; d[i] = z;
    }
}
int zero_planes4(float *const p[4], size_t n, hipStream_t s)
{
    if ((n & 3) || (((uintptr_t)p[0] | (uintptr_t)p[1] | (uintptr_t)p[2] | (uintptr_t)p[3]) & 15)) {
        for (int j = 0; j < 4; ++j) MI_HIP_TRY(hipMemsetAsync(p[j], 0, sizeof(float) * n, s));
        return MI_OK;
    }
    const long long n4 = (long long)(n / 4);
    const int blocks = (int)std::min<long long>((n4 + 255) / 256, 2048);
    hipLaunchKernelGGL(k_zero4, dim3(std::max(blocks, 1)), dim3(256), 0, s, (float4 *)p[0], (float4 *)p[1], (float4 *)p[2], (float4 *)p[3], n4);
    MI_HIP_TRY(hipGetLastError());
    return MI_OK;
}

int unpack_flow(const PtrTab *tab, float *u1, float *u2, const Geo &g, hipStream_t s)
{
    hipLaunchKernelGGL(k_unpack_flow, grid2d(g, g.batch), dim3(256), 0, s, tab, u1, u2, g);
    MI_HIP_TRY(hipGetLastError());
    return MI_OK;
}

int pack_flow(const PtrTab *tab, const float *u1[2], const float *u2[2], const Geo &g, const Ctl *ctl,
              int cur_host, hipStream_t s)
{
    hipLaunchKernelGGL(k_pack_flow, grid2d(g, g.batch), dim3(256), 0, s, tab, u1[0], u1[1], u2[0], u2[1], g,
                       make_ctlk(ctl), cur_host);
    MI_HIP_TRY(hipGetLastError());
    return MI_OK;
}

int resize(int semantics, int nplanes, const float *const src[3][2], int src_sets, float *const dst[3],
           const Geo &gs, const Geo &gd, double inv_scale_x, double inv_scale_y, const float post_scale[3],
           const Ctl *ctl, int cur_host, hipStream_t s)
{
    ResizeArgs A;
    memset(&A, 0, sizeof(A));
    for (int i = 0; i < 3; ++i) {
        A.src[i][0] = i < nplanes ? src[i][0] : nullptr;
        A.src[i][1] = i < nplanes ? src[i][src_sets == 2 ? 1 : 0] : nullptr;
        A.dst[i] = i < nplanes ? dst[i] : nullptr;
        A.post[i] = i < nplanes ? post_scale[i] : 1.f;
    }
    A.nsets = src_sets;
    A.nplanes = nplanes;
    A.gs = gs;
    A.gd = gd;
    const CtlK ck = make_ctlk(ctl);
#define MI_RSZ(SEMV, PX, ROWS) hipLaunchKernelGGL((k_resize<SEMV, PX, ROWS>), dim3(div_up(gd.w, 64 * PX), div_up(gd.h, 4 * ROWS), nplanes * gd.batch), dim3(256), 0, s, A, ck, cur_host)
    if (semantics == MI_SEM_CPU_REF) {
        A.scale_x = 1.0 / inv_scale_x;
        A.scale_y = 1.0 / inv_scale_y;
        MI_RSZ(MI_SEM_CPU_REF, 1, RSZ_ROWS);
    } else {
        A.scale_x = (double)(float)(1.0 / inv_scale_x);
        A.scale_y = (double)(float)(1.0 / inv_scale_y);
        MI_RSZ(MI_SEM_CUDA_COMPAT, 1, RSZ_ROWS);
    }
#undef MI_RSZ
    MI_HIP_TRY(hipGetLastError());
    return MI_OK;
}

int median_flow(int ksize, float *const u1[2], float *const u2[2], float *tmp1, float *tmp2, const Geo &g, const Ctl *ctl, int cur_host,
                hipStream_t s)
{
    MedArgs A;
    A.u[0][0] = u1[0]; A.u[1][0] = u1[1]; A.u[0][1] = u2[0]; A.u[1][1] = u2[1];
    A.tmp[0] = tmp1; A.tmp[1] = tmp2; A.g = g;
    const CtlK ck = make_ctlk(ctl);
    const dim3 grid(div_up(g.w, 64), div_up(g.h, 4), g.batch * 2);
    if (ksize == 5) hipLaunchKernelGGL(k_median<5>, grid, dim3(256), 0, s, A, ck, cur_host);
    else if (ksize == 3) hipLaunchKernelGGL(k_median<3>, grid, dim3(256), 0, s, A, ck, cur_host);
    else { set_error("medianFiltering must be 1 (off), 3 or 5 for CV_32F (cv::medianBlur)"); return MI_ERR_BAD_ARG; }
    hipLaunchKernelGGL(k_median_copy, grid, dim3(256), 0, s, A, ck, cur_host);
    MI_HIP_TRY(hipGetLastError());
    return MI_OK;
}

int gradient(const float *src, float *dx, float *dy, const Geo &g, hipStream_t s)
{
    hipLaunchKernelGGL(k_gradient, grid2d(g, g.batch), dim3(256), 0, s, src, dx, dy, g);
    MI_HIP_TRY(hipGetLastError());
    return MI_OK;
}

int pack3(const float *a, const float *b, const float *c, float *pk, const Geo &g, hipStream_t s)
{
    hipLaunchKernelGGL(k_pack3, grid2d(g, g.batch), dim3(256), 0, s, a, b, c, reinterpret_cast<float4 *>(pk), g);
    MI_HIP_TRY(hipGetLastError());
    return MI_OK;
}

int warp(int semantics, const float *I0, const float *pk, const float *u1[2], const float *u2[2], float *I1w,
         float *I1wx, float *I1wy, float *grad, float *rho, const float *cubic_tab_dev, const Geo &g, const Ctl *ctl,
         int cur_host, hipStream_t s)
{
    WarpArgs A;
    A.I0 = I0; A.pk = reinterpret_cast<const float4 *>(pk);
    A.u1[0] = u1[0]; A.u1[1] = u1[1]; A.u2[0] = u2[0]; A.u2[1] = u2[1];
    A.I1w = I1w; A.I1wx = I1wx; A.I1wy = I1wy; A.grad = grad; A.rho = rho;
    A.tab = cubic_tab_dev;
    A.g = g;
    const CtlK ck = make_ctlk(ctl);
    if (semantics == MI_SEM_CPU_REF) {
#ifdef MIFLOW_EXPERIMENTS
        const int tile = warp_tile();
        if (tile == 16)
            hipLaunchKernelGGL((k_warp<MI_SEM_CPU_REF, 16>), dim3(div_up(g.w, 16), div_up(g.h, 16), g.batch), dim3(256), 0, s, A, ck, cur_host);
        else if (tile == 64)
            hipLaunchKernelGGL((k_warp<MI_SEM_CPU_REF, 64>), grid2d(g, g.batch), dim3(256), 0, s, A, ck, cur_host);
        else
#endif
            hipLaunchKernelGGL((k_warp<MI_SEM_CPU_REF, 32>), dim3(div_up(g.w, 32), div_up(g.h, 8), g.batch), dim3(256), 0, s, A, ck, cur_host);
    } else
        hipLaunchKernelGGL(k_warp<MI_SEM_CUDA_COMPAT>, grid2d(g, g.batch), dim3(256), 0, s, A, ck, cur_host);
    MI_HIP_TRY(hipGetLastError());
    return MI_OK;
}

static int pick_rows_per_wave(const Geo &g)
{
    const int strips = div_up(g.w, STRIP_W);
    int R = 32;
    while (R > 8 && (long long)strips * div_up(g.h, R) * g.batch < 4096) R >>= 1;
    return R;
}

template <bool EXACT, bool PZ>
static void launch_iter(const IterArgs &A, const dim3 grid, const Ctl *ctl, int cur_host, hipStream_t s)
{
    const CtlK ck = make_ctlk(ctl);
    const bool check = ctl && ctl->S;
    if (A.pl.gamma != 0.f) {
        if (check) hipLaunchKernelGGL((k_iterate<EXACT, PZ, true, true>), grid, dim3(256), 0, s, A, ck, cur_host);
        else hipLaunchKernelGGL((k_iterate<EXACT, PZ, false, true>), grid, dim3(256), 0, s, A, ck, cur_host);
        return;
    }
    if (check)
        hipLaunchKernelGGL((k_iterate<EXACT, PZ, true>), grid, dim3(256), 0, s, A, ck, cur_host);
    else
        hipLaunchKernelGGL((k_iterate<EXACT, PZ, false>), grid, dim3(256), 0, s, A, ck, cur_host);
}

int iterate(bool exact, const IterPlanes &pl, const Geo &g, float l_t, float theta, float taut, bool p_zero,
            const Ctl *ctl, int cur_host, hipStream_t s)
{
    IterArgs A;
    A.pl = pl;
    A.g = g;
    A.l_t = l_t; A.theta = theta; A.taut = taut;
    A.rows_per_wave = pick_rows_per_wave(g);
    const dim3 grid(div_up(g.w, STRIP_W), div_up(div_up(g.h, A.rows_per_wave), 4), g.batch);
    if (exact) { if (p_zero) launch_iter<true, true>(A, grid, ctl, cur_host, s); else launch_iter<true, false>(A, grid, ctl, cur_host, s); }
    else       { if (p_zero) launch_iter<false, true>(A, grid, ctl, cur_host, s); else launch_iter<false, false>(A, grid, ctl, cur_host, s); }
    MI_HIP_TRY(hipGetLastError());
    return MI_OK;
}

void host_cubic_table(float tab[128])
{
    const float A = -0.75f, scale = 1.f / 32;
    for (int i = 0; i < 32; ++i) {
        const float x = (float)i * scale;
        float *c = tab + i * 4;
        c[0] = ((A * (x + 1) - 5 * A) * (x + 1) + 8 * A) * (x + 1) - 4 * A;
        c[1] = ((A + 2) * x - (A + 3)) * x * x + 1;
        c[2] = ((A + 2) * (1 - x) - (A + 3)) * (1 - x) * (1 - x) + 1;
        c[3] = 1.f - c[0] - c[1] - c[2];
    }
}

}
}
```

opencv_contrib_amd/csrc/tvl1_plan.h:

```cpp
#pragma once
#include "miflow/c_api.h"
#include "tvl1_tb_table.h"
#include <algorithm>
#include <array>
#include <cmath>
#include <cstddef>
#include <initializer_list>
#include <vector>

namespace mi {
namespace tvl1 {

struct Geo {
    int w, h, ld;
    long long ps;
    int batch;
};

constexpr int kTbMaxBlock = 10;
constexpr int kTbExactMaxBlock = 5;
constexpr int kTileMaxBlock = 10;
constexpr double kLargeLevel = 12e6;

struct TvKnobs {
    long long tile_maxpx;
    int tile_spec;
    int tile_variant, tile_small_wgs, tile_variants, tile_rows[8];
    int tile_fb_block, tile_fb_model;
    bool tb_force;
    int tb_nograd, tb_jw, tb_jw_spec;
    int tb_ppl, tb_wps, tb_pf;
    int tb_p16;
    int tb_il;
    int tb_fw;
    int tb_skip_p, tb_hist, spec, exact_tb;
    int fb_poll, fb_ahead;
    int warp_fast, warp_lds, x_skip;
};


inline bool tile_eligible(const Geo &g, const TvKnobs &K)
{
    return K.tile_maxpx > 0 && (long long)g.w * g.h * g.batch <= K.tile_maxpx;
}
inline bool runs_on_tiles(const Geo &g, int T, const TvKnobs &K, bool spec = false)
{
    return tile_eligible(g, K) && T <= kTileMaxBlock && (spec ? K.tile_spec != 0 : !K.tb_force);
}

enum class TbUse { Fixed, Indep, Exact, Spec };

inline const TbRow *tb_select(TbUse use, int T, bool gam, bool nograd, const TvKnobs &K, int fw = 0)
{
    const int mode = use == TbUse::Spec ? 1 : use == TbUse::Exact ? 2 : 0;
    const auto first = [&](auto pred) -> const TbRow * {
        for (const TbRow &r : kTbRows)
            if (r.MODE == mode && r.T == T && r.GAM == gam && (r.FW != 0) == (fw != 0) && pred(r)) return &r;
        return nullptr;
    };
    const auto any = [](const TbRow &) { return true; };
    const auto indep = [](const TbRow &r) { return r.JW == 0 && !r.NG; };
    if (use == TbUse::Exact) return gam || nograd ? nullptr : first(any);
    if (use == TbUse::Indep) return nograd ? nullptr : gam ? first([](const TbRow &r) { return r.JW == 0; }) : first(indep);
    if (gam) return first(any);
    if (use == TbUse::Spec) {
        const TbRow *reads = nograd ? nullptr : (K.tb_jw >= 2 && K.tb_jw_spec) ? first([](const TbRow &r) { return r.JW == 2 && !r.NG; }) : first(indep);
        return reads ? reads : first([](const TbRow &r) { return r.NG; });
    }
    if (fw) return first([&](const TbRow &r) { return r.FW == fw; });
    if (nograd) return first([&](const TbRow &r) { return r.NG && r.P16 == (K.tb_p16 != 0); });
    if (K.tb_jw && K.tb_ppl < 0)
        if (const TbRow *joined = first([&](const TbRow &r) { return r.JW == K.tb_jw && !r.NG; })) return joined;
    const TbRow *variant = first([&](const TbRow &r) { return indep(r) && r.PPL == K.tb_ppl && r.WPS == K.tb_wps && r.PF == K.tb_pf; });
    return variant ? variant : first(indep);
}

struct TbKernel {
    bool tile;
    const TbRow *row;
    int rows;
};
struct TbOverride {
    bool force_streaming;
    int rows;
    bool independent_waves;
};
inline TbKernel tb_kernel(TbUse use, int T, const Geo &g, bool gam, bool nograd, const TvKnobs &K, const TbOverride &o = TbOverride{})
{
    if (!o.force_streaming && (use == TbUse::Fixed || use == TbUse::Spec) && runs_on_tiles(g, T, K, use == TbUse::Spec))
        return TbKernel{true, nullptr, 0};
    return TbKernel{false, tb_select(o.independent_waves ? TbUse::Indep : use, T, gam, nograd, K), o.rows};
}

inline bool tb_nograd_ok(int T, const Geo &g, const TvKnobs &K)
{
    return K.tb_nograd && K.tb_jw == 2 && K.tb_ppl < 0 && !runs_on_tiles(g, T, K) && tb_select(TbUse::Fixed, T, false, true, K);
}
inline bool tb_spec_nograd_ok(const Geo &g, const TvKnobs &K)
{
    return K.tb_nograd && K.tb_jw >= 2 && K.tb_jw_spec && !(tile_eligible(g, K) && K.tile_spec != 0);
}
inline bool tb_fused_ok(int T, const Geo &g, int semantics, bool fast_warp, const TvKnobs &K)
{
    if (!K.tb_fw || !tb_nograd_ok(T, g, K) || g.w < 6 || g.h < 6) return false;
    return (semantics == MI_SEM_CPU_REF && !fast_warp) || (semantics == MI_SEM_CUDA_COMPAT && fast_warp);
}

inline int tile_auto_variant(const Geo &g, bool spec, const TvKnobs &K)
{
    if (K.tile_variant >= 0) return K.tile_variant < K.tile_variants ? K.tile_variant : 0;
    constexpr int M = kTileMaxBlock, LW = 64, STRIDE = LW - 2 * M;
    const long long nstrips = g.w <= LW - M ? 1 : 1 + (g.w - (LW - M) + STRIDE - 1) / STRIDE;
    const long long wgs = nstrips * ((g.h + (64 - 2 * M) - 1) / (64 - 2 * M)) * g.batch;
    return wgs < (long long)K.tile_small_wgs * (spec ? 2 : 1) ? 1 : 0;
}
inline int tile_rows_for(const Geo &g, const TvKnobs &K) { return K.tile_rows[tile_auto_variant(g, true, K)]; }

inline std::vector<int> greedy_blocks(int n, int cap, std::initializer_list<int> sup)
{
    std::vector<int> blocks;
    for (int left = n; left > 0; left -= blocks.back()) {
        int t = 1;
        for (int c : sup) if (c <= left && c <= cap) t = std::max(t, c);
        blocks.push_back(t);
    }
    return blocks;
}
inline std::vector<int> tb_plan(int n, int cap, const TvKnobs &K)
{
    static const int sup[] = {1, 2, 3, 4, 5, 6, 8, 10};
    static const double cost[11] = {0, 15.6, 9.4, 6.6, 4.65, 3.9, 3.7, 0, 2.83, 0, 2.54};
    std::vector<int> blocks;
    if (n <= 0) return blocks;
    if (K.tb_force) return greedy_blocks(n, cap, {1, 2, 3, 4, 5, 6, 8, 10});
    std::vector<double> best(n + 1, 1e300);
    std::vector<int> pick(n + 1, 1);
    best[0] = 0;
    for (int i = 1; i <= n; ++i)
        for (int t : sup) {
            if (t > i || t > cap) continue;
            const double c = best[i - t] + t * cost[t];
            if (c < best[i]) { best[i] = c; pick[i] = t; }
        }
    for (int i = n; i > 0; i -= pick[i]) blocks.push_back(pick[i]);
    return blocks;
}
inline std::vector<int> tb_plan_level(const Geo &g, int n, int cap, bool gam, const TvKnobs &K)
{
    if (!tile_eligible(g, K) || K.tb_force) return gam ? greedy_blocks(n, cap, {10, 5, 2, 1}) : tb_plan(n, cap, K);
    return greedy_blocks(n, std::min(cap, kTileMaxBlock), {1, 2, 3, 4, 5, 6, 7, 8, 9, 10});
}
inline std::vector<int> tb_spec_plan(int n, int list, int B, const TvKnobs &K)
{
    std::vector<int> blocks;
    const int want = n + (n > 10 ? 30 : n > 1 ? 10 : 0);
    const int tile = (B <= 2 && K.tile_fb_block > 0) ? std::min(K.tile_fb_block, kTileMaxBlock) : kTileMaxBlock;
    for (int sum = 0; sum < want; sum += blocks.back())
        blocks.push_back(list == 3 ? tile : n <= 5 ? 5 : list == 0 ? 10 : blocks.size() < 12 ? 5 : 10);
    return blocks;
}

struct TbBandShape {
    int T, PF, H;
    long long per_band;
    long long cap;
    long long simds;
    int wps;
};
inline long long tb_band_wave_steps(int T, int PF, int rows)
{
    const int P = T + 1 + PF;
    return (long long)((rows + 2 * T + P - 1) / P) * P;
}
inline long long tb_band_sum_steps(int T, int PF, int H, int R)
{
    const int nb = (H + R - 1) / R;
    return (nb - 1) * tb_band_wave_steps(T, PF, R) + tb_band_wave_steps(T, PF, H - (nb - 1) * R);
}
inline int tb_band_count(const TbBandShape &b)
{
    long long best_cost = -1;
    int best_nb = 1;
    for (int nb = 1; nb <= b.H; ++nb) {
        const int R = (b.H + nb - 1) / nb;
        if (R < 8 && nb > 1) break;
        const long long cap_nb = b.simds > 0 && nb < 4 && nb < b.wps ? b.simds * nb : b.cap;
        const long long rounds = (b.per_band * nb + cap_nb - 1) / cap_nb;
        const long long cost = rounds * tb_band_wave_steps(b.T, b.PF, R);
        if (best_cost < 0 || cost < best_cost) { best_cost = cost; best_nb = nb; }
    }
    return best_nb;
}
inline int tb_band_rows_equal(const TbBandShape &b) { const int nb = tb_band_count(b); return (b.H + nb - 1) / nb; }
inline int tb_band_rows(const TbBandShape &b)
{
    const int nb = tb_band_count(b);
    const int R0 = (b.H + nb - 1) / nb;
    if (nb == 1) return R0;
    const long long tallest = tb_band_wave_steps(b.T, b.PF, R0);
    int best = R0;
    long long best_sum = tb_band_sum_steps(b.T, b.PF, b.H, R0);
    for (int R = R0 + 1; (long long)(nb - 1) * R < b.H; ++R) {
        if (tb_band_wave_steps(b.T, b.PF, R) > tallest) break;
        const long long sum = tb_band_sum_steps(b.T, b.PF, b.H, R);
        if (sum < best_sum) { best_sum = sum; best = R; }
    }
    return best;
}


struct TvShape {
    int W, H, B, type;
    mi_tvl1_params P;
    int lanes;
    bool capturing;
};

enum class TvForm {
    Blocked,
    ExactBlocked,
    Spec,
    PerIter,
};

struct TvWarp {
    TvForm form;
    std::vector<int> blocks;
    std::vector<TbKernel> run;
    int outer;
    bool on_tiles;
    bool nograd;
    bool fused;
    bool warp_launch;
    bool skip_iterations;
    bool skip_p_last;
    bool pack_in_pass;
};

constexpr size_t kNoPlane = (size_t)-1;
struct TvArena {
    size_t total = 0;
    std::vector<std::array<size_t, 8>> lv;
    size_t scr[6];
    size_t p[12];
};

struct TvPlan {
    std::vector<Geo> geo;
    int used;
    TvArena arena;
    int iters;
    int median;
    bool check, spec, hist;
    bool fb, fb_poll;
    bool fast_warp;
    long long Q;
    unsigned long long hist_sig;
    std::vector<std::vector<TvWarp>> warp;
};

inline std::vector<Geo> tv_levels(const mi_tvl1_params &P, int W, int H, int B, int *used)
{
    std::vector<Geo> geo;
    int w = W, h = H;
    *used = 0;
    for (int s = 0; s < P.nscales; ++s) {
        if (s > 0) {
            w = (int)std::lrint(w * P.scale_step);
            h = (int)std::lrint(h * P.scale_step);
            if (w < 1 || h < 1) break;
        }
        geo.push_back(Geo{w, h, (w + 63) / 64 * 64, (long long)((w + 63) / 64 * 64) * h, B});
        if (s > 0 && (w < 16 || h < 16)) break;
        *used = s + 1;
    }
    return geo;
}

inline TvArena tv_arena(const std::vector<Geo> &geo, int B, bool gam, bool med)
{
    TvArena a;
    auto take = [&](size_t nfloats) { const size_t o = a.total; a.total += (nfloats + 63) / 64 * 64; return o; };
    for (const Geo &g : geo) {
        const size_t n = (size_t)g.ps * B;
        std::array<size_t, 8> o;
        o[0] = take(n); o[1] = take(n);
        for (int k = 0; k < 6; ++k) o[2 + k] = (k % 3 == 2 && !gam) ? kNoPlane : take(n);
        a.lv.push_back(o);
    }
    const size_t nfull = (size_t)geo[0].ps * B;
    for (int k = 0; k < 6; ++k) a.scr[k] = (k < 2 && !med) ? kNoPlane : take(nfull);
    for (int k = 0; k < 12; ++k) a.p[k] = (k % 6 >= 4 && !gam) ? kNoPlane : take(nfull);
    return a;
}

inline int spec_tile_block(int hprev, const Geo &g, const TvKnobs &K)
{
    const double px = (double)g.w * g.h * g.batch, TR = (double)tile_rows_for(g, K);
    int best = 10;
    double best_cost = 1e30;
    for (int bl : {4, 7, 10}) {
        const double passes = (double)((hprev + bl - 1) / bl);
        const double lanes = px * 64.0 / (64.0 - 2.0 * bl) * TR / (TR - 2.0 * bl);
        const double cost = passes * (double)K.tile_fb_model + lanes * (passes * 10.8e-6 + (double)hprev * 2.4e-6);
        if (cost < best_cost) { best_cost = cost; best = bl; }
    }
    return best;
}
inline std::vector<int> spec_blocks(const TvWarp &w, const Geo &g, int hprev, const TvKnobs &K, int bl = 0)
{
    std::vector<int> plan = w.blocks;
    if (!w.on_tiles || hprev < 1 || plan.empty()) return plan;
    if (K.tile_fb_model != 0) {
        if (bl <= 0) bl = spec_tile_block(hprev, g, K);
        int total = 0;
        for (int v : plan) total += v;
        plan.assign((size_t)((total + bl - 1) / bl), bl);
    } else if (hprev <= 7) plan[0] = hprev <= 4 ? 4 : 7;
    return plan;
}
inline int spec_first_poll(const std::vector<int> &plan, int hprev, int prev_done)
{
    if (hprev <= 0) return std::max(1, prev_done);
    int kq = 0, sum = 0;
    while (kq < (int)plan.size() && (sum += plan[kq]) < hprev) ++kq;
    return std::max(1, std::min(kq + 1, (int)plan.size() - 1));
}
inline void spec_hist_fraction(int wp, int *num, int *den)
{
    *num = wp == 0 ? 7 : wp == 1 ? 9 : 4;
    *den = wp == 0 ? 10 : wp == 1 ? 20 : 5;
}

inline TvPlan tv_make_plan(const TvShape &S, const TvKnobs &K)
{
    const mi_tvl1_params &P = S.P;
    const int B = S.B;
    const bool gam = P.gamma != 0.0;
    TvPlan p;
    p.geo = tv_levels(P, S.W, S.H, B, &p.used);
    p.median = P.median_filtering > 1 ? P.median_filtering : 0;
    p.arena = tv_arena(p.geo, B, gam, p.median != 0);
    p.iters = P.iterations * P.inner_iterations;
    p.check = P.epsilon > 0.0 && p.iters > 0;
    p.spec = p.check && !P.exact_math && P.time_block != 1 && !p.median && K.spec != 0;
    p.hist = p.spec && K.tb_hist != 0;
    p.fb = p.spec && S.lanes == 1 && P.host_feedback >= 0 && (P.host_feedback == 1 || B <= 2) && !S.capturing;
    p.fb_poll = p.fb && K.fb_poll != 0;
    p.fast_warp = !P.exact_math && (K.warp_fast > 0 || (K.warp_fast < 0 && P.semantics == MI_SEM_CUDA_COMPAT));
    p.hist_sig = 1469598103934665603ull;
    for (long long v : {(long long)S.W, (long long)S.H, (long long)B, (long long)p.used, (long long)P.warps, (long long)p.iters, (long long)S.type})
        p.hist_sig = (p.hist_sig ^ (unsigned long long)v) * 1099511628211ull;

    const long long sw = (long long)p.used * P.warps;
    p.Q = sw * p.iters;
    std::vector<int> spec_list[4];
    if (p.spec) {
        long long e_max = 0, l_max = 0;
        for (int k = 0; k < 4; ++k) {
            spec_list[k] = tb_spec_plan(p.iters, k, B, K);
            long long t = 0;
            for (int v : spec_list[k]) t += v;
            e_max = std::max(e_max, t);
            l_max = std::max(l_max, (long long)spec_list[k].size() + 1);
        }
        e_max += 2 * (long long)std::max(kTileMaxBlock, kTbMaxBlock);
        p.Q = std::max(sw * e_max, sw * l_max);
    }

    const bool blocked = !p.check && !P.exact_math && P.time_block != 1;
    const bool exact_blocked = !p.check && P.exact_math && P.time_block != 1 && !gam && !p.median && K.exact_tb != 0;
    p.warp.resize(p.used);
    for (int s = 0; s < p.used; ++s) {
        const Geo &g = p.geo[s];
        TvWarp w{};
        w.outer = 1;
        if (blocked) {
            w.form = TvForm::Blocked;
            w.outer = p.median ? P.iterations : 1;
            w.blocks = tb_plan_level(g, p.median ? P.inner_iterations : p.iters, P.time_block > 0 ? P.time_block : kTbMaxBlock, gam, K);
            w.nograd = !w.blocks.empty();
            for (int v : w.blocks) w.nograd = w.nograd && (gam || tb_nograd_ok(v, g, K));
            for (int v : w.blocks) w.run.push_back(tb_kernel(TbUse::Fixed, v, g, gam, w.nograd, K));
            w.fused = !gam && w.nograd && w.blocks.size() == 1 && !p.median && K.x_skip == 0 && K.warp_lds == 0 &&
                      tb_fused_ok(w.blocks[0], g, P.semantics, p.fast_warp, K);
            if (w.fused) w.run[0].row = tb_select(TbUse::Fixed, w.blocks[0], false, true, K, P.semantics == MI_SEM_CPU_REF ? 1 : 2);
            w.skip_iterations = K.x_skip == 2;
        } else if (exact_blocked) {
            w.form = TvForm::ExactBlocked;
            const int cap = P.time_block > 0 ? std::min(P.time_block, kTbExactMaxBlock) : kTbExactMaxBlock;
            for (int left = p.iters; left > 0; left -= w.blocks.back()) w.blocks.push_back(std::min(left, cap));
            for (int v : w.blocks) w.run.push_back(tb_kernel(TbUse::Exact, v, g, false, false, K));
        } else if (p.spec) {
            w.form = TvForm::Spec;
            w.nograd = gam || tb_spec_nograd_ok(g, K);
        } else
            w.form = TvForm::PerIter;
        p.warp[s].assign(P.warps, w);
        for (int wp = 0; wp < P.warps; ++wp) {
            TvWarp &x = p.warp[s][wp];
            if (x.form == TvForm::Spec) {
                x.on_tiles = tb_kernel(TbUse::Spec, kTileMaxBlock, g, gam, x.nograd, K).tile;
                x.blocks = spec_list[x.on_tiles ? 3 : wp > 0 ? 2 : ((double)g.w * g.h * B >= kLargeLevel ? 0 : 1)];
                for (int v : x.blocks) x.run.push_back(tb_kernel(TbUse::Spec, v, g, gam, x.nograd, K));
            }
            x.warp_launch = !x.fused && !(K.x_skip == 1 && wp > 0);
            x.skip_p_last = x.form == TvForm::Blocked && K.tb_skip_p && wp == P.warps - 1 && !p.median;
            if (s == 0 && x.skip_p_last && !gam && !x.fused && !x.skip_iterations && !P.use_initial_flow && !x.blocks.empty())
                x.pack_in_pass = K.tb_il != 0 && x.run.back().row && tb_il_form(*x.run.back().row);
        }
    }
    return p;
}

}
}
```

opencv_contrib_amd/csrc/tvl1_warp_dev.h:

```cpp
#pragma once
#include "tvl1_dev.h"

namespace mi {
namespace tvl1 {

struct CtlK {
    int2 *S;
    unsigned long long *E;
    int Q, q, q_prev, first_of_warp, reset_cur;
    double thr;
    double *P;
    int sched, n, need_done;
};
static inline CtlK make_ctlk(const Ctl *c)
{
    CtlK k;
    memset(&k, 0, sizeof(k));
    k.q_prev = -1;
    if (c) { k.S = c->S; k.E = c->E; k.Q = c->Q; k.q = c->q; k.q_prev = c->q_prev;
             k.first_of_warp = c->first_of_warp; k.reset_cur = c->reset_cur; k.thr = c->thr;
             k.P = c->P; k.sched = c->sched; k.n = c->n; k.need_done = c->need_done; }
    return k;
}
__device__ __forceinline__ bool warp_gate_k(const CtlK &c, int b)
{
    if (!c.S || !c.need_done || c.q_prev < 0) return true;
    return (c.S[(long long)b * c.Q + c.q_prev].y & MI_SLOT_DONE) != 0;
}
__device__ __forceinline__ int resolve_cur_k(const CtlK &c, int b, int cur_host)
{
    if (!c.S) return cur_host;
    if (c.q_prev < 0) return 0;
    const int2 s = c.S[(long long)b * c.Q + c.q_prev];
    return s.x ^ (s.y & 1);
}

struct Warp6Args {
    const float *I0, *I1;
    const float *u1[2], *u2[2];
    float *I1w, *I1wx, *I1wy, *grad, *rho;
    const float *tab;
    Geo g;
    int swz;
};

static inline int warp_tile() { return tuning().warp_tile; }

}
}
```

opencv_contrib_amd/csrc/tvl1_warp_kernels.hip:

```cpp
#include "tvl1_dev.h"
#include "tvl1_warp_dev.h"
#include "tvl1_warp_px.h"

namespace mi {
namespace tvl1 {

template <int SEM, int TX, int NP, bool FAST>
__global__ __launch_bounds__(256) void k_warp6(Warp6Args A, CtlK ctl, int cur_host)
{
    __shared__ float s_tab[128];
    if (SEM == MI_SEM_CPU_REF) {
        if (threadIdx.x < 128) s_tab[threadIdx.x] = A.tab[threadIdx.x];
        __syncthreads();
    }
    constexpr int TY = 64 / TX;
    const int lane_ = threadIdx.x & 63, wave_ = threadIdx.x >> 6;
    unsigned bx = blockIdx.x, by = blockIdx.y, bz = blockIdx.z;
    if (A.swz) {
        const unsigned nwg = gridDim.x * gridDim.y, orig = by * gridDim.x + bx;
        const unsigned xcd = orig & 7u, qq = nwg >> 3, rr = nwg & 7u;
        const unsigned lid = (xcd < rr ? xcd * (qq + 1) : rr * (qq + 1) + (xcd - rr) * qq) + (orig >> 3);
        by = lid / gridDim.x; bx = lid - by * gridDim.x;
    }
    const int x0 = (int)bx * (TX * NP) + (lane_ % TX);
    const int y = (int)by * (4 * TY) + wave_ * TY + lane_ / TX;
    const int b = (int)bz;
    const int W = A.g.w, H = A.g.h, ld = A.g.ld;
    if (x0 >= W || y >= H) return;
    if (!warp_gate_k(ctl, b)) return;
    const int cur = resolve_cur_k(ctl, b, cur_host);
    const long long pb = (long long)b * A.g.ps;
    const long long orow = pb + (long long)y * ld;
    const float *U1 = A.u1[cur] + orow, *U2 = A.u2[cur] + orow, *I0r = A.I0 + orow;
    const float *P = A.I1 + pb;
    float i0n = I0r[x0], u1n = U1[x0], u2n = U2[x0];
#pragma unroll
    for (int i = 0; i < NP; ++i) {
        const int x = x0 + i * TX;
        if (x >= W) break;
        const float u1v = u1n, u2v = u2n, i0 = i0n;
        if (i + 1 < NP) {
            const int xn = min(x + TX, W - 1);
            u1n = U1[xn]; u2n = U2[xn];
            i0n = I0r[xn];
        }
        warp_px<SEM, FAST>(A, s_tab, P, x, y, orow + x, u1v, u2v, i0);
    }
}

#ifdef MIFLOW_EXPERIMENTS
constexpr int WL_TW = 64, WL_TH = 16, WL_PPT = 4;
constexpr int WL_RW = 96, WL_RH = 40;

template <int SEM, bool FAST>
__global__ __launch_bounds__(256) void k_warp_lds(Warp6Args A, CtlK ctl, int cur_host)
{
    __shared__ __attribute__((aligned(16))) float s_reg[WL_RH * WL_RW];
    __shared__ float s_tab[128];
    __shared__ int s_mm[4];
    if (SEM == MI_SEM_CPU_REF && threadIdx.x < 128) s_tab[threadIdx.x] = A.tab[threadIdx.x];
    if (threadIdx.x == 0) { s_mm[0] = 0x7fffffff; s_mm[1] = -0x7fffffff; s_mm[2] = 0x7fffffff; s_mm[3] = -0x7fffffff; }
    const int lane = threadIdx.x & 63, wave = threadIdx.x >> 6;
    const int W = A.g.w, H = A.g.h, ld = A.g.ld;
    const int x = blockIdx.x * WL_TW + lane;
    const int yb = blockIdx.y * WL_TH + wave * WL_PPT;
    const int b = blockIdx.z;
    if (!warp_gate_k(ctl, b)) return;
    const int cur = resolve_cur_k(ctl, b, cur_host);
    const long long pb = (long long)b * A.g.ps;
    const float *P = A.I1 + pb;
    const int xc = min(x, W - 1);
    float u1v[WL_PPT], u2v[WL_PPT], i0[WL_PPT];
#pragma unroll
    for (int k = 0; k < WL_PPT; ++k) {
        const long long o = pb + (long long)min(yb + k, H - 1) * ld + xc;
        u1v[k] = A.u1[cur][o]; u2v[k] = A.u2[cur][o]; i0[k] = A.I0[o];
    }
    __syncthreads();
    int mn_x = 0x7fffffff, mx_x = -0x7fffffff, mn_y = 0x7fffffff, mx_y = -0x7fffffff;
#pragma unroll
    for (int k = 0; k < WL_PPT; ++k) {
        int sx, sy;
        float wxv[4], wyv[4];
        warp_coords<SEM>(s_tab, x, yb + k, u1v[k], u2v[k], sx, sy, wxv, wyv);
        const bool interior = (unsigned)(sx - 1) < (unsigned)max(W - 5, 0) && (unsigned)(sy - 1) < (unsigned)max(H - 5, 0);
        if (interior && x < W && yb + k < H) { mn_x = min(mn_x, sx); mx_x = max(mx_x, sx); mn_y = min(mn_y, sy); mx_y = max(mx_y, sy); }
    }
#pragma unroll
    for (int o = 32; o > 0; o >>= 1) {
        mn_x = min(mn_x, __shfl_xor(mn_x, o)); mx_x = max(mx_x, __shfl_xor(mx_x, o));
        mn_y = min(mn_y, __shfl_xor(mn_y, o)); mx_y = max(mx_y, __shfl_xor(mx_y, o));
    }
    if (lane == 0) { atomicMin(&s_mm[0], mn_x); atomicMax(&s_mm[1], mx_x); atomicMin(&s_mm[2], mn_y); atomicMax(&s_mm[3], mx_y); }
    __syncthreads();
    const int rx0 = (s_mm[0] - 1) & ~3, ry0 = s_mm[2] - 1;
    const int rw = s_mm[1] + 4 - rx0 + 1, rh = s_mm[3] + 4 - ry0 + 1;
    const bool staged = s_mm[1] >= s_mm[0] && rw <= WL_RW && rh <= WL_RH;
    if (staged) {
        const int rw4 = (rw + 3) >> 2;
        for (int idx = threadIdx.x; idx < rh * (WL_RW / 4); idx += 256) {
            const int r = idx / (WL_RW / 4), c4 = idx - r * (WL_RW / 4);
            if (c4 < rw4) {
                const float4 v = *reinterpret_cast<const float4 *>(P + (long long)(ry0 + r) * ld + rx0 + 4 * c4);
                *reinterpret_cast<float4 *>(&s_reg[r * WL_RW + 4 * c4]) = v;
            }
        }
    }
    __syncthreads();
    if (x >= W) return;
#pragma unroll 1
    for (int k = 0; k < WL_PPT; ++k) {
        const int y = yb + k;
        if (y >= H) break;
        const long long o = pb + (long long)y * ld + x;
        int sx, sy;
        float wxv[4], wyv[4];
        warp_coords<SEM>(s_tab, x, y, u1v[k], u2v[k], sx, sy, wxv, wyv);
        const bool interior = (unsigned)(sx - 1) < (unsigned)max(W - 5, 0) && (unsigned)(sy - 1) < (unsigned)max(H - 5, 0);
        if (!(staged && interior)) {
            warp_px<SEM, FAST>(A, s_tab, P, x, y, o, u1v[k], u2v[k], i0[k]);
            continue;
        }
        float R[6][6];
        const float *q = &s_reg[(sy - 1 - ry0) * WL_RW + (sx - 1 - rx0)];
#pragma unroll
        for (int r = 0; r < 6; ++r)
#pragma unroll
            for (int c = 0; c < 6; ++c)
                if (!((r == 0 || r == 5) && (c == 0 || c == 5))) R[r][c] = q[r * WL_RW + c];
        float v0, v1, v2;
        window_sums<SEM, FAST>(R, wxv, wyv, v0, v1, v2);
        if (A.I1w) A.I1w[o] = v0;
        A.I1wx[o] = v1;
        A.I1wy[o] = v2;
        if (A.grad) A.grad[o] = v1 * v1 + v2 * v2;
        A.rho[o] = (v0 - v1 * u1v[k] - v2 * u2v[k] - i0[k]);
    }
}

#endif

int warp_fused(int semantics, bool fast, int lds, const float *I0, const float *I1, const float *u1[2], const float *u2[2], float *I1w, float *I1wx,
               float *I1wy, float *grad, float *rho, const float *cubic_tab_dev, const Geo &g, const Ctl *ctl, int cur_host,
               hipStream_t s)
{
    Warp6Args A;
    A.I0 = I0; A.I1 = I1; A.swz = tuning().warp_swz != 0 ? 1 : 0;
    A.u1[0] = u1[0]; A.u1[1] = u1[1]; A.u2[0] = u2[0]; A.u2[1] = u2[1];
    A.I1w = I1w; A.I1wx = I1wx; A.I1wy = I1wy; A.grad = grad; A.rho = rho;
    A.tab = cubic_tab_dev;
    A.g = g;
    const CtlK ck = make_ctlk(ctl);
    const bool cpu = semantics == MI_SEM_CPU_REF;
    if (lds < 0 ? tuning().warp_lds != 0 : lds != 0) {
#ifndef MIFLOW_EXPERIMENTS
        set_error("the LDS-staged warp (k_warp_lds) exists in the experiments build only (-DMIFLOW_EXPERIMENTS)");
        return MI_ERR_NOT_IMPL;
#else
        const dim3 grid(div_up(g.w, WL_TW), div_up(g.h, WL_TH), g.batch);
        if (cpu && fast) hipLaunchKernelGGL((k_warp_lds<MI_SEM_CPU_REF, true>), grid, dim3(256), 0, s, A, ck, cur_host);
        else if (cpu) hipLaunchKernelGGL((k_warp_lds<MI_SEM_CPU_REF, false>), grid, dim3(256), 0, s, A, ck, cur_host);
        else if (fast) hipLaunchKernelGGL((k_warp_lds<MI_SEM_CUDA_COMPAT, true>), grid, dim3(256), 0, s, A, ck, cur_host);
        else hipLaunchKernelGGL((k_warp_lds<MI_SEM_CUDA_COMPAT, false>), grid, dim3(256), 0, s, A, ck, cur_host);
        MI_HIP_TRY(hipGetLastError());
        return MI_OK;
#endif
    }
#ifndef MIFLOW_EXPERIMENTS
    {
        const dim3 grid(div_up(g.w, 32 * 2), div_up(g.h, 4 * 2), g.batch);
        if (cpu && fast) hipLaunchKernelGGL((k_warp6<MI_SEM_CPU_REF, 32, 2, true>), grid, dim3(256), 0, s, A, ck, cur_host);
        else if (cpu) hipLaunchKernelGGL((k_warp6<MI_SEM_CPU_REF, 32, 2, false>), grid, dim3(256), 0, s, A, ck, cur_host);
        else if (fast) hipLaunchKernelGGL((k_warp6<MI_SEM_CUDA_COMPAT, 32, 2, true>), grid, dim3(256), 0, s, A, ck, cur_host);
        else hipLaunchKernelGGL((k_warp6<MI_SEM_CUDA_COMPAT, 32, 2, false>), grid, dim3(256), 0, s, A, ck, cur_host);
        MI_HIP_TRY(hipGetLastError());
        return MI_OK;
    }
#else
    const int tile = warp_tile();
    const int np = tuning().warp_np;
    const dim3 grid(div_up(g.w, tile * np), div_up(g.h, 4 * (64 / tile)), g.batch);
#define LAUNCH_W6T(SEM, TX, NP)                                                                                          \
    do {                                                                                                                 \
        if (fast) hipLaunchKernelGGL((k_warp6<SEM, TX, NP, true>), grid, dim3(256), 0, s, A, ck, cur_host);              \
        else hipLaunchKernelGGL((k_warp6<SEM, TX, NP, false>), grid, dim3(256), 0, s, A, ck, cur_host);                  \
    } while (0)
#define LAUNCH_W6N(SEM, NP)                                                                                              \
    do {                                                                                                                 \
        if (tile == 16) LAUNCH_W6T(SEM, 16, NP); else if (tile == 32) LAUNCH_W6T(SEM, 32, NP); else LAUNCH_W6T(SEM, 64, NP); \
    } while (0)
#define LAUNCH_W6(SEM)                                                                                                   \
    do {                                                                                                                 \
        if (np == 1) LAUNCH_W6N(SEM, 1); else if (np == 4) LAUNCH_W6N(SEM, 4); else LAUNCH_W6N(SEM, 2);                    \
    } while (0)
    if (cpu) LAUNCH_W6(MI_SEM_CPU_REF);
    else LAUNCH_W6(MI_SEM_CUDA_COMPAT);
#undef LAUNCH_W6T
#undef LAUNCH_W6N
#undef LAUNCH_W6
    MI_HIP_TRY(hipGetLastError());
    return MI_OK;
#endif
}

}
}
```

opencv_contrib_amd/csrc/tvl1_warp_px.h:

```cpp
#pragma once
#include "tvl1_dev.h"
#include "tvl1_warp_dev.h"

namespace mi {
namespace tvl1 {

typedef float f4u __attribute__((ext_vector_type(4), aligned(4)));
typedef float f2u __attribute__((ext_vector_type(2), aligned(4)));

__device__ __forceinline__ float bicubic_coeff_cuda6(float x_)
{
    const float x = fabsf(x_);
    if (x <= 1.0f) return x * x * (1.5f * x - 2.5f) + 1.0f;
    else if (x < 2.0f) return x * (x * (-0.5f * x + 2.5f) - 4.0f) + 2.0f;
    return 0.0f;
}

__device__ __forceinline__ void fetch3(const float *P, int W, int H, int ld, int cx, int cy, float &v, float &vx, float &vy)
{
    const float *row = P + (long long)cy * ld;
    v = row[cx];
    vx = 0.5f * (row[min(cx + 1, W - 1)] - row[max(cx - 1, 0)]);
    vy = 0.5f * (P[(long long)min(cy + 1, H - 1) * ld + cx] - P[(long long)max(cy - 1, 0) * ld + cx]);
}

template <int SEM, bool FAST>
__device__ __forceinline__ void window_sums(const float (&R)[6][6], const float (&wxv)[4], const float (&wyv)[4], float &v0, float &v1,
                                            float &v2)
{
    if (FAST) {
        float a[6], bx[4];
#pragma unroll
        for (int r = 0; r < 6; ++r)
            a[r] = fmaf(wxv[3], R[r][4], fmaf(wxv[2], R[r][3], fmaf(wxv[1], R[r][2], wxv[0] * R[r][1])));
        const float d2 = wxv[0] - wxv[2], d3 = wxv[1] - wxv[3];
#pragma unroll
        for (int r = 1; r < 5; ++r)
            bx[r - 1] = fmaf(wxv[3], R[r][5], fmaf(wxv[2], R[r][4], fmaf(d3, R[r][3], fmaf(d2, R[r][2], fmaf(-wxv[1], R[r][1], -wxv[0] * R[r][0])))));
        float s0 = fmaf(wyv[3], a[4], fmaf(wyv[2], a[3], fmaf(wyv[1], a[2], wyv[0] * a[1])));
        float s1 = fmaf(wyv[3], bx[3], fmaf(wyv[2], bx[2], fmaf(wyv[1], bx[1], wyv[0] * bx[0])));
        float s2 = fmaf(wyv[3], a[5] - a[3], fmaf(wyv[2], a[4] - a[2], fmaf(wyv[1], a[3] - a[1], wyv[0] * (a[2] - a[0]))));
        if (SEM == MI_SEM_CUDA_COMPAT) {
            const float coeff = __builtin_amdgcn_rcpf(((wxv[0] + wxv[1]) + (wxv[2] + wxv[3])) * ((wyv[0] + wyv[1]) + (wyv[2] + wyv[3])));
            s0 *= coeff; s1 *= coeff; s2 *= coeff;
        }
        v0 = s0; v1 = 0.5f * s1; v2 = 0.5f * s2;
    } else if (SEM == MI_SEM_CPU_REF) {
        float s0 = 0.f, s1 = 0.f, s2 = 0.f;
#pragma unroll
        for (int j = 0; j < 4; ++j) {
            float t0[4], t1[4], t2[4], w[4];
#pragma unroll
            for (int i = 0; i < 4; ++i) {
                w[i] = wyv[j] * wxv[i];
                t0[i] = R[j + 1][i + 1];
                t1[i] = R[j + 1][i + 2] - R[j + 1][i];
                t2[i] = R[j + 2][i + 1] - R[j][i + 1];
            }
            const float r0 = t0[0] * w[0] + t0[1] * w[1] + t0[2] * w[2] + t0[3] * w[3];
            const float r1 = t1[0] * w[0] + t1[1] * w[1] + t1[2] * w[2] + t1[3] * w[3];
            const float r2 = t2[0] * w[0] + t2[1] * w[1] + t2[2] * w[2] + t2[3] * w[3];
            if (j == 0) { s0 = r0; s1 = r1; s2 = r2; } else { s0 += r0; s1 += r1; s2 += r2; }
        }
        v0 = s0; v1 = 0.5f * s1; v2 = 0.5f * s2;
    } else {
        float sum = 0.f, sumx = 0.f, sumy = 0.f, wsum = 0.f;
#pragma unroll
        for (int j = 0; j < 4; ++j)
#pragma unroll
            for (int i = 0; i < 4; ++i) {
                const float wgt = wxv[i] * wyv[j];
                sum += wgt * R[j + 1][i + 1];
                sumx += wgt * (R[j + 1][i + 2] - R[j + 1][i]);
                sumy += wgt * (R[j + 2][i + 1] - R[j][i + 1]);
                wsum += wgt;
            }
        const float coeff = 1.0f / wsum;
        v0 = sum * coeff; v1 = (0.5f * sumx) * coeff; v2 = (0.5f * sumy) * coeff;
    }
}

__device__ __forceinline__ void fetch3b(__amdgpu_buffer_rsrc_t rs, int W, int H, int ld, int cx, int cy, float &v, float &vx, float &vy)
{
    const unsigned ro = (unsigned)cy * (unsigned)ld;
    const auto L = [&](unsigned e) { return __uint_as_float(__builtin_amdgcn_raw_buffer_load_b32(rs, 4u * e, 0, 0)); };
    v = L(ro + cx);
    vx = 0.5f * (L(ro + min(cx + 1, W - 1)) - L(ro + max(cx - 1, 0)));
    vy = 0.5f * (L((unsigned)min(cy + 1, H - 1) * (unsigned)ld + cx) - L((unsigned)max(cy - 1, 0) * (unsigned)ld + cx));
}

template <int SEM>
__device__ __forceinline__ void warp_coords(const float *s_tab, int x, int y, float u1v, float u2v, int &sx, int &sy, float (&wxv)[4],
                                            float (&wyv)[4])
{
    if (SEM == MI_SEM_CPU_REF) {
        const float mx = (float)x + u1v, my = (float)y + u2v;
        const int qx = __float2int_rn(mx * 32.0f), qy = __float2int_rn(my * 32.0f);
        sx = min(max(qx >> 5, -32768), 32767) - 1;
        sy = min(max(qy >> 5, -32768), 32767) - 1;
#pragma unroll
        for (int k = 0; k < 4; ++k) { wxv[k] = s_tab[(qx & 31) * 4 + k]; wyv[k] = s_tab[(qy & 31) * 4 + k]; }
    } else {
        const float wxp = (float)x + u1v, wyp = (float)y + u2v;
        sx = (int)fminf(fmaxf(floorf(wxp), -1.0e9f), 1.0e9f) - 1;
        sy = (int)fminf(fmaxf(floorf(wyp), -1.0e9f), 1.0e9f) - 1;
#pragma unroll
        for (int k = 0; k < 4; ++k) {
            wxv[k] = bicubic_coeff_cuda6(wxp - (float)(sx + k));
            wyv[k] = bicubic_coeff_cuda6(wyp - (float)(sy + k));
        }
    }
}

__device__ __forceinline__ bool window_interior(int sx, int sy, int W, int H)
{
    return (unsigned)(sx - 1) < (unsigned)max(W - 5, 0) && (unsigned)(sy - 1) < (unsigned)max(H - 5, 0);
}
__device__ __forceinline__ void window_gather(float (&R)[6][6], const float *P, int ld, int sx, int sy)
{
    const float *q = P + (long long)(sy - 1) * ld + (sx - 1);
    {
        const f4u a = *reinterpret_cast<const f4u *>(q + 1);
        R[0][1] = a.x; R[0][2] = a.y; R[0][3] = a.z; R[0][4] = a.w;
    }
#pragma unroll
    for (int r = 1; r < 5; ++r) {
        const float *qr = q + (long long)r * ld;
        const f4u a = *reinterpret_cast<const f4u *>(qr);
        const f2u c = *reinterpret_cast<const f2u *>(qr + 4);
        R[r][0] = a.x; R[r][1] = a.y; R[r][2] = a.z; R[r][3] = a.w; R[r][4] = c.x; R[r][5] = c.y;
    }
    {
        const f4u a = *reinterpret_cast<const f4u *>(q + (long long)5 * ld + 1);
        R[5][1] = a.x; R[5][2] = a.y; R[5][3] = a.z; R[5][4] = a.w;
    }
}

template <int SEM>
__device__ __forceinline__ void window_border(const float *P, int W, int H, int ld, int sx, int sy, const float (&wxv)[4], const float (&wyv)[4],
                                              float &v0, float &v1, float &v2)
{
    if (SEM == MI_SEM_CPU_REF) {
        const __amdgpu_buffer_rsrc_t rs = __builtin_amdgcn_make_buffer_rsrc(const_cast<float *>(P), 0, (unsigned)H * (unsigned)ld * 4u, 0x00020000);
        const auto L = [&](unsigned e) { return __uint_as_float(__builtin_amdgcn_raw_buffer_load_b32(rs, 4u * e, 0, 0)); };
        unsigned cxs[6];
#pragma unroll
        for (int c = 0; c < 6; ++c) cxs[c] = (unsigned)min(max(sx - 1 + c, 0), W - 1);
        const bool win4 = (unsigned)sx < (unsigned)max(W - 3, 0) && (unsigned)sy < (unsigned)max(H - 3, 0);
        float s0 = 0.f, s1 = 0.f, s2 = 0.f, b0 = 0.f, b1 = 0.f, b2 = 0.f;
#pragma unroll 1
        for (int j = 0; j < 4; ++j) {
            const int yj = sy + j;
            const unsigned ra = (unsigned)min(max(yj - 1, 0), H - 1) * (unsigned)ld, rb = (unsigned)min(max(yj, 0), H - 1) * (unsigned)ld,
                           rc = (unsigned)min(max(yj + 1, 0), H - 1) * (unsigned)ld;
            float Ra[4], Rb[6], Rc[4];
#pragma unroll
            for (int c = 0; c < 6; ++c) Rb[c] = L(rb + cxs[c]);
#pragma unroll
            for (int c = 0; c < 4; ++c) { Ra[c] = L(ra + cxs[c + 1]); Rc[c] = L(rc + cxs[c + 1]); }
            const float wyj = j == 0 ? wyv[0] : j == 1 ? wyv[1] : j == 2 ? wyv[2] : wyv[3];
            float t0[4], t1[4], t2[4], w[4];
            const bool okj = (unsigned)yj < (unsigned)H;
#pragma unroll
            for (int i = 0; i < 4; ++i) {
                w[i] = wyj * wxv[i];
                t0[i] = Rb[i + 1];
                t1[i] = 0.5f * (Rb[i + 2] - Rb[i]);
                t2[i] = 0.5f * (Rc[i] - Ra[i]);
            }
            const float r0 = t0[0] * w[0] + t0[1] * w[1] + t0[2] * w[2] + t0[3] * w[3];
            const float r1 = t1[0] * w[0] + t1[1] * w[1] + t1[2] * w[2] + t1[3] * w[3];
            const float r2 = t2[0] * w[0] + t2[1] * w[1] + t2[2] * w[2] + t2[3] * w[3];
            if (j == 0) { s0 = r0; s1 = r1; s2 = r2; } else { s0 += r0; s1 += r1; s2 += r2; }
#pragma unroll
            for (int i = 0; i < 4; ++i) {
                const bool ok = okj && (unsigned)(sx + i) < (unsigned)W;
                const float n0 = b0 + (t0[i] - 0.f) * w[i], n1 = b1 + (t1[i] - 0.f) * w[i], n2 = b2 + (t2[i] - 0.f) * w[i];
                b0 = ok ? n0 : b0; b1 = ok ? n1 : b1; b2 = ok ? n2 : b2;
            }
        }
        v0 = win4 ? s0 : b0; v1 = win4 ? s1 : b1; v2 = win4 ? s2 : b2;
    } else {
        const __amdgpu_buffer_rsrc_t rs = __builtin_amdgcn_make_buffer_rsrc(const_cast<float *>(P), 0, (unsigned)H * (unsigned)ld * 4u, 0x00020000);
        float sum = 0.f, sumx = 0.f, sumy = 0.f, wsum = 0.f;
#pragma unroll 1
        for (int j = 0; j < 4; ++j) {
            const int cy = sy + j;
            const float wyj = j == 0 ? wyv[0] : j == 1 ? wyv[1] : j == 2 ? wyv[2] : wyv[3];
            float t0[4], t1[4], t2[4];
#pragma unroll
            for (int i = 0; i < 4; ++i) fetch3b(rs, W, H, ld, min(max(sx + i, 0), W - 1), min(max(cy, 0), H - 1), t0[i], t1[i], t2[i]);
#pragma unroll
            for (int i = 0; i < 4; ++i) {
                const float wgt = wxv[i] * wyj;
                sum += wgt * t0[i];
                sumx += wgt * t1[i];
                sumy += wgt * t2[i];
                wsum += wgt;
            }
        }
        const float coeff = 1.0f / wsum;
        v0 = sum * coeff; v1 = sumx * coeff; v2 = sumy * coeff;
    }
}

template <int SEM, bool FAST>
__device__ __forceinline__ void warp_px(const Warp6Args &A, const float *s_tab, const float *P, int x, int y, long long o, float u1v,
                                        float u2v, float i0)
{
    const int W = A.g.w, H = A.g.h, ld = A.g.ld;
    int sx, sy;
    float wxv[4], wyv[4];
    warp_coords<SEM>(s_tab, x, y, u1v, u2v, sx, sy, wxv, wyv);

    float v0, v1, v2;
    if (window_interior(sx, sy, W, H)) {
        float R[6][6];
        window_gather(R, P, ld, sx, sy);
        window_sums<SEM, FAST>(R, wxv, wyv, v0, v1, v2);
    } else {
        window_border<SEM>(P, W, H, ld, sx, sy, wxv, wyv, v0, v1, v2);
    }
    if (A.I1w) A.I1w[o] = v0;
    A.I1wx[o] = v1;
    A.I1wy[o] = v2;
    const float Ix2 = v1 * v1, Iy2 = v2 * v2;
    if (A.grad) A.grad[o] = Ix2 + Iy2;
    A.rho[o] = (v0 - v1 * u1v - v2 * u2v - i0);
}

}
}
```

Baseline: 1488 pairs/s.

## Read f32 input frames in place instead of converting to device planes

Result: no change. 1503 pairs/s (median of 6 runs) (+1.0%).

```diff
diff --git a/opencv_contrib_amd/csrc/mi_common.cpp b/opencv_contrib_amd/csrc/mi_common.cpp
--- a/opencv_contrib_amd/csrc/mi_common.cpp
+++ b/opencv_contrib_amd/csrc/mi_common.cpp
@@ -72,6 +72,7 @@
         t.tb_rows = EXP_INT("MIFLOW_TB_ROWS", 0);
         t.tb_rows_equal = EXP_INT("MIFLOW_TB_ROWS_EQUAL", 0);
         t.tb_il = EXP_INT("MIFLOW_TB_IL", 1);
+        t.f32_in_place = EXP_INT("MIFLOW_F32_IN_PLACE", 1);
         t.tb_verbose = getenv("MIFLOW_TB_VERBOSE") != nullptr;
         {
             const char *e = getenv("MIFLOW_TILE_MAXPX");
diff --git a/opencv_contrib_amd/csrc/mi_common.h b/opencv_contrib_amd/csrc/mi_common.h
--- a/opencv_contrib_amd/csrc/mi_common.h
+++ b/opencv_contrib_amd/csrc/mi_common.h
@@ -49,6 +49,7 @@
     int tb_plan_wps;
     int tb_rows;
     int tb_rows_equal;
+    int f32_in_place;
     int tb_il;
     int tb_verbose;
     long long tile_maxpx;
diff --git a/opencv_contrib_amd/csrc/tvl1_api.cpp b/opencv_contrib_amd/csrc/tvl1_api.cpp
--- a/opencv_contrib_amd/csrc/tvl1_api.cpp
+++ b/opencv_contrib_amd/csrc/tvl1_api.cpp
@@ -278,8 +278,10 @@
         v.tile_fb_block = t.tile_fb_block; v.tile_fb_model = t.tile_fb_model;
         v.tb_force = t.tb_force != 0; v.tb_nograd = t.tb_nograd; v.tb_jw = t.tb_jw; v.tb_jw_spec = t.tb_jw_spec;
         v.tb_ppl = t.tb_ppl; v.tb_wps = t.tb_wps; v.tb_pf = t.tb_pf; v.tb_p16 = t.tb_p16; v.tb_il = t.tb_il;
+        v.f32_in_place = t.f32_in_place;
         v.tb_fw = t.tb_fw; v.tb_skip_p = t.tb_skip_p; v.tb_hist = t.tb_hist; v.spec = t.spec; v.exact_tb = t.exact_tb;
         v.fb_poll = t.fb_poll; v.fb_ahead = t.fb_ahead; v.warp_fast = t.warp_fast; v.warp_lds = t.warp_lds; v.x_skip = t.x_skip;
+        v.warp_shape_variant = (t.warp_tile != 32 || t.warp_np != 2) ? 1 : 0;
         return v;
     }();
     return k;
@@ -345,6 +347,7 @@
     int q_settle_prev = -1, q_settle_scale = -1;
     int fb_prev_warp = 2, fb_prev_scale = 2;
     int cur = 0;
+    bool frames_in_place = false;
     bool first_of_scale = true;
     bool pre_warped = false;
 };
@@ -366,7 +369,7 @@
     const mi_tvl1_params &P = r.h->P;
     Lane &ln = r.ln;
     const int ns = r.pl.used, B = r.B;
-    int rc = convert(ln.tab.p, type, ln.L[0].I0, ln.L[0].I1, ln.L[0].g, r.st);
+    int rc = r.frames_in_place ? MI_OK : convert(ln.tab.p, type, ln.L[0].I0, ln.L[0].I1, ln.L[0].g, r.st);
     if (rc) return rc;
     if (P.use_initial_flow && (rc = unpack_flow(ln.tab.p, ln.L[0].u[0][0], ln.L[0].u[0][1], ln.L[0].g, r.st))) return rc;
     const float one3[3] = {1.f, 1.f, 1.f};
@@ -374,7 +377,8 @@
         const LevelBuf &c = ln.L[s - 1];
         const float *src[3][2] = {{c.I0, nullptr}, {c.I1, nullptr}, {nullptr, nullptr}};
         float *dst[3] = {ln.L[s].I0, ln.L[s].I1, nullptr};
-        rc = resize(P.semantics, 2, src, 1, dst, c.g, ln.L[s].g, P.scale_step, P.scale_step, one3, nullptr, 0, r.st);
+        rc = resize(P.semantics, 2, src, 1, dst, c.g, ln.L[s].g, P.scale_step, P.scale_step, one3, nullptr, 0, r.st,
+                    s == 1 && r.frames_in_place ? ln.tab.p : nullptr);
         if (rc) return rc;
         if ((int)s >= ns) break;
         if (P.use_initial_flow) {
@@ -402,8 +406,10 @@
     c.q_prev = r.q_last;
     c.need_done = ahead ? 1 : 0;
     const bool dev_cur = ahead || (r.pl.check && !r.first_of_scale);
+    const bool level0 = &Lv == &r.ln.L[0];
     return warp_fused(r.h->P.semantics, r.pl.fast_warp, -1, Lv.I0, Lv.I1, u1v, u2v, nullptr, r.ln.scr[2], r.ln.scr[3],
-                      r.grad, r.ln.scr[5], r.h->cubic_tab.p, Lv.g, dev_cur ? &c : nullptr, r.cur, r.st);
+                      r.grad, r.ln.scr[5], r.h->cubic_tab.p, Lv.g, dev_cur ? &c : nullptr, r.cur, r.st,
+                      level0 && r.frames_in_place ? r.ln.tab.p : nullptr);
 }
 
 int run_blocked(Run &r, LevelBuf &Lv, const TvWarp &w, long long *nlaunch)
@@ -669,6 +675,9 @@
     r.ctl.S = ln.S.p; r.ctl.E = ln.E.p; r.ctl.Q = (int)ln.Q; r.ctl.P = ln.Pd.p;
     r.ctl.sched = P.semantics == MI_SEM_CUDA_COMPAT ? 1 : 0;
     r.l_t = (float)(P.lambda * P.theta); r.taut = (float)(P.tau / P.theta); r.theta = (float)P.theta;
+    r.frames_in_place = pl.frames_in_place;
+    for (int i = 0; i < n && r.frames_in_place; ++i)
+        r.frames_in_place = (unsigned long long)I0s[i].step * I0s[i].rows < (1ull << 32) && (unsigned long long)I1s[i].step * I1s[i].rows < (1ull << 32);
     if ((rc = enqueue_pyramid(r, I0s[0].type))) return rc;
     for (int s = pl.used - 1; s >= 0; --s) {
         LevelBuf &Lv = ln.L[s];
diff --git a/opencv_contrib_amd/csrc/tvl1_dev.h b/opencv_contrib_amd/csrc/tvl1_dev.h
--- a/opencv_contrib_amd/csrc/tvl1_dev.h
+++ b/opencv_contrib_amd/csrc/tvl1_dev.h
@@ -48,7 +48,7 @@
               const Ctl *ctl, int cur_host, hipStream_t s);
 int resize(int semantics, int nplanes, const float *const src[3][2], int src_sets, float *const dst[3],
            const Geo &gs, const Geo &gd, double inv_scale_x, double inv_scale_y,
-           const float post_scale[3], const Ctl *ctl, int cur_host, hipStream_t s);
+           const float post_scale[3], const Ctl *ctl, int cur_host, hipStream_t s, const PtrTab *frames = nullptr);
 int gradient(const float *src, float *dx, float *dy, const Geo &g, hipStream_t s);
 int median_flow(int ksize, float *const u1[2], float *const u2[2], float *tmp1, float *tmp2, const Geo &g, const Ctl *ctl, int cur_host,
                 hipStream_t s);
@@ -58,7 +58,7 @@
          int cur_host, hipStream_t s);
 int warp_fused(int semantics, bool fast, int lds, const float *I0, const float *I1, const float *u1[2], const float *u2[2], float *I1w, float *I1wx,
                float *I1wy, float *grad, float *rho, const float *cubic_tab_dev, const Geo &g, const Ctl *ctl, int cur_host,
-               hipStream_t s);
+               hipStream_t s, const PtrTab *frames = nullptr);
 int iterate(bool exact, const IterPlanes &pl, const Geo &g, float l_t, float theta, float taut,
             bool p_zero, const Ctl *ctl, int cur_host, hipStream_t s);
 
diff --git a/opencv_contrib_amd/csrc/tvl1_kernels.hip b/opencv_contrib_amd/csrc/tvl1_kernels.hip
--- a/opencv_contrib_amd/csrc/tvl1_kernels.hip
+++ b/opencv_contrib_amd/csrc/tvl1_kernels.hip
@@ -127,10 +127,11 @@
     int nsets, nplanes;
     Geo gs, gd;
     double scale_x, scale_y;
+    const PtrTab *frames;
 };
 
 #define RSZ_ROWS 8
-template <int SEM, int PX, int ROWS>
+template <int SEM, int PX, int ROWS, bool TAB = false>
 __global__ __launch_bounds__(256) void k_resize(ResizeArgs A, CtlK ctl, int cur_host)
 {
     const int dx = (blockIdx.x * 64 + (threadIdx.x & 63)) * PX;
@@ -138,8 +139,14 @@
     const int pl = blockIdx.z % A.nplanes, b = blockIdx.z / A.nplanes;
     if (dx >= A.gd.w || dy0 >= A.gd.h) return;
     const int cur = A.nsets == 2 ? resolve_cur_k(ctl, b, cur_host) : 0;
-    const float *S = A.src[pl][cur] + (long long)b * A.gs.ps;
-    const int sw = A.gs.w, sh = A.gs.h, ld = A.gs.ld;
+    const float *S = TAB ? nullptr : A.src[pl][cur] + (long long)b * A.gs.ps;
+    const int sw = A.gs.w, sh = A.gs.h;
+    int ld = A.gs.ld;
+    if constexpr (TAB) {
+        const PtrTab t = A.frames[b];
+        S = reinterpret_cast<const float *>(pl == 0 ? t.a : t.b);
+        ld = (int)((pl == 0 ? t.step_a : t.step_b) >> 2);
+    }
     const float ps = A.post[pl];
     RszX X[PX];
 #pragma unroll
@@ -150,11 +157,22 @@
         const int dy = dy0 + r;
         if (dy >= A.gd.h) break;
         const RszX Y = resize_yside<SEM>(dy, sh, A.scale_y);
-        const float *R0 = S + (long long)Y.i0 * ld, *R1 = S + (long long)Y.i1 * ld;
+        const float *R0 = S + (long long)(TAB ? min(Y.i0, sh - 1) : Y.i0) * ld, *R1 = S + (long long)Y.i1 * ld;
         float o[PX];
 #pragma unroll
         for (int j = 0; j < PX; ++j) {
-            o[j] = resize_combine<SEM>(R0, R1, X[j], Y);
+            if constexpr (TAB) {
+                typedef const __attribute__((address_space(1))) char *gcchar_ptr;
+                typedef const __attribute__((address_space(1))) float *gcfloat_ptr;
+                const gcfloat_ptr G0 = reinterpret_cast<gcfloat_ptr>((gcchar_ptr) reinterpret_cast<const char *>(R0));
+                const gcfloat_ptr G1 = reinterpret_cast<gcfloat_ptr>((gcchar_ptr) reinterpret_cast<const char *>(R1));
+                const int c0 = min(X[j].i0, sw - 1), c1 = X[j].i1;
+                const float t0[2] = {G0[c0] * 255.0f, G0[c1] * 255.0f}, t1[2] = {G1[c0] * 255.0f, G1[c1] * 255.0f};
+                const RszX X2{0, 1, X[j].w0, X[j].w1};
+                o[j] = resize_combine<SEM>(t0, t1, X2, Y);
+            } else {
+                o[j] = resize_combine<SEM>(R0, R1, X[j], Y);
+            }
             if (ps != 1.0f) o[j] = o[j] * ps;
         }
         if (PX == 4) *reinterpret_cast<float4 *>(D + (long long)dy * A.gd.ld) = make_float4(o[0], o[1], o[2], o[3]);
@@ -639,10 +657,12 @@
 
 int resize(int semantics, int nplanes, const float *const src[3][2], int src_sets, float *const dst[3],
            const Geo &gs, const Geo &gd, double inv_scale_x, double inv_scale_y, const float post_scale[3],
-           const Ctl *ctl, int cur_host, hipStream_t s)
-{
+           const Ctl *ctl, int cur_host, hipStream_t s, const PtrTab *frames)
+{
+    MI_REQUIRE(!frames || (nplanes == 2 && src_sets == 1), MI_ERR_BAD_ARG, "frames in place: the two planes of the pyramid's first resize");
     ResizeArgs A;
     memset(&A, 0, sizeof(A));
+    A.frames = frames;
     for (int i = 0; i < 3; ++i) {
         A.src[i][0] = i < nplanes ? src[i][0] : nullptr;
         A.src[i][1] = i < nplanes ? src[i][src_sets == 2 ? 1 : 0] : nullptr;
@@ -655,16 +675,18 @@
     A.gd = gd;
     const CtlK ck = make_ctlk(ctl);
 #define MI_RSZ(SEMV, PX, ROWS) hipLaunchKernelGGL((k_resize<SEMV, PX, ROWS>), dim3(div_up(gd.w, 64 * PX), div_up(gd.h, 4 * ROWS), nplanes * gd.batch), dim3(256), 0, s, A, ck, cur_host)
+#define MI_RSZ_TAB(SEMV, PX, ROWS) hipLaunchKernelGGL((k_resize<SEMV, PX, ROWS, true>), dim3(div_up(gd.w, 64 * PX), div_up(gd.h, 4 * ROWS), nplanes * gd.batch), dim3(256), 0, s, A, ck, cur_host)
     if (semantics == MI_SEM_CPU_REF) {
         A.scale_x = 1.0 / inv_scale_x;
         A.scale_y = 1.0 / inv_scale_y;
-        MI_RSZ(MI_SEM_CPU_REF, 1, RSZ_ROWS);
+        if (frames) MI_RSZ_TAB(MI_SEM_CPU_REF, 1, RSZ_ROWS); else MI_RSZ(MI_SEM_CPU_REF, 1, RSZ_ROWS);
     } else {
         A.scale_x = (double)(float)(1.0 / inv_scale_x);
         A.scale_y = (double)(float)(1.0 / inv_scale_y);
-        MI_RSZ(MI_SEM_CUDA_COMPAT, 1, RSZ_ROWS);
+        if (frames) MI_RSZ_TAB(MI_SEM_CUDA_COMPAT, 1, RSZ_ROWS); else MI_RSZ(MI_SEM_CUDA_COMPAT, 1, RSZ_ROWS);
     }
 #undef MI_RSZ
+#undef MI_RSZ_TAB
     MI_HIP_TRY(hipGetLastError());
     return MI_OK;
 }
diff --git a/opencv_contrib_amd/csrc/tvl1_plan.h b/opencv_contrib_amd/csrc/tvl1_plan.h
--- a/opencv_contrib_amd/csrc/tvl1_plan.h
+++ b/opencv_contrib_amd/csrc/tvl1_plan.h
@@ -33,9 +33,11 @@
     int tb_p16;
     int tb_il;
     int tb_fw;
+    int f32_in_place;
     int tb_skip_p, tb_hist, spec, exact_tb;
     int fb_poll, fb_ahead;
     int warp_fast, warp_lds, x_skip;
+    int warp_shape_variant;
 };
 
 
@@ -209,6 +211,11 @@
 }
 
 
+inline bool tv_frames_in_place(int type, const TvKnobs &K)
+{
+    return type == MI_32FC1 && K.f32_in_place != 0 && K.tb_fw == 0 && K.warp_lds == 0 && K.warp_shape_variant == 0;
+}
+
 struct TvShape {
     int W, H, B, type;
     mi_tvl1_params P;
@@ -254,6 +261,7 @@
     bool check, spec, hist;
     bool fb, fb_poll;
     bool fast_warp;
+    bool frames_in_place;
     long long Q;
     unsigned long long hist_sig;
     std::vector<std::vector<TvWarp>> warp;
@@ -347,6 +355,7 @@
     p.hist = p.spec && K.tb_hist != 0;
     p.fb = p.spec && S.lanes == 1 && P.host_feedback >= 0 && (P.host_feedback == 1 || B <= 2) && !S.capturing;
     p.fb_poll = p.fb && K.fb_poll != 0;
+    p.frames_in_place = tv_frames_in_place(S.type, K);
     p.fast_warp = !P.exact_math && (K.warp_fast > 0 || (K.warp_fast < 0 && P.semantics == MI_SEM_CUDA_COMPAT));
     p.hist_sig = 1469598103934665603ull;
     for (long long v : {(long long)S.W, (long long)S.H, (long long)B, (long long)p.used, (long long)P.warps, (long long)p.iters, (long long)S.type})
diff --git a/opencv_contrib_amd/csrc/tvl1_warp_dev.h b/opencv_contrib_amd/csrc/tvl1_warp_dev.h
--- a/opencv_contrib_amd/csrc/tvl1_warp_dev.h
+++ b/opencv_contrib_amd/csrc/tvl1_warp_dev.h
@@ -42,6 +42,7 @@
     const float *tab;
     Geo g;
     int swz;
+    const PtrTab *frames;
 };
 
 static inline int warp_tile() { return tuning().warp_tile; }
diff --git a/opencv_contrib_amd/csrc/tvl1_warp_kernels.hip b/opencv_contrib_amd/csrc/tvl1_warp_kernels.hip
--- a/opencv_contrib_amd/csrc/tvl1_warp_kernels.hip
+++ b/opencv_contrib_amd/csrc/tvl1_warp_kernels.hip
@@ -5,7 +5,7 @@
 namespace mi {
 namespace tvl1 {
 
-template <int SEM, int TX, int NP, bool FAST>
+template <int SEM, int TX, int NP, bool FAST, bool INPL = false>
 __global__ __launch_bounds__(256) void k_warp6(Warp6Args A, CtlK ctl, int cur_host)
 {
     __shared__ float s_tab[128];
@@ -33,7 +33,15 @@
     const long long orow = pb + (long long)y * ld;
     const float *U1 = A.u1[cur] + orow, *U2 = A.u2[cur] + orow, *I0r = A.I0 + orow;
     const float *P = A.I1 + pb;
-    float i0n = I0r[x0], u1n = U1[x0], u2n = U2[x0];
+    int ldP = ld;
+    if constexpr (INPL) {
+        const PtrTab t = A.frames[b];
+        I0r = reinterpret_cast<const float *>(reinterpret_cast<const char *>(t.a) + (long long)y * t.step_a);
+        P = reinterpret_cast<const float *>(t.b);
+        ldP = (int)(t.step_b >> 2);
+    }
+    const auto load_i0 = [&](int xx) { return INPL ? frame_load<INPL, float>(I0r + xx) * kFrameScale : I0r[xx]; };
+    float i0n = load_i0(x0), u1n = U1[x0], u2n = U2[x0];
 #pragma unroll
     for (int i = 0; i < NP; ++i) {
         const int x = x0 + i * TX;
@@ -42,9 +50,9 @@
         if (i + 1 < NP) {
             const int xn = min(x + TX, W - 1);
             u1n = U1[xn]; u2n = U2[xn];
-            i0n = I0r[xn];
+            i0n = load_i0(xn);
         }
-        warp_px<SEM, FAST>(A, s_tab, P, x, y, orow + x, u1v, u2v, i0);
+        warp_px<SEM, FAST, INPL>(A, s_tab, P, ldP, x, y, orow + x, u1v, u2v, i0);
     }
 }
 
@@ -118,7 +126,7 @@
         warp_coords<SEM>(s_tab, x, y, u1v[k], u2v[k], sx, sy, wxv, wyv);
         const bool interior = (unsigned)(sx - 1) < (unsigned)max(W - 5, 0) && (unsigned)(sy - 1) < (unsigned)max(H - 5, 0);
         if (!(staged && interior)) {
-            warp_px<SEM, FAST>(A, s_tab, P, x, y, o, u1v[k], u2v[k], i0[k]);
+            warp_px<SEM, FAST>(A, s_tab, P, ld, x, y, o, u1v[k], u2v[k], i0[k]);
             continue;
         }
         float R[6][6];
@@ -142,16 +150,28 @@
 
 int warp_fused(int semantics, bool fast, int lds, const float *I0, const float *I1, const float *u1[2], const float *u2[2], float *I1w, float *I1wx,
                float *I1wy, float *grad, float *rho, const float *cubic_tab_dev, const Geo &g, const Ctl *ctl, int cur_host,
-               hipStream_t s)
+               hipStream_t s, const PtrTab *frames)
 {
     Warp6Args A;
     A.I0 = I0; A.I1 = I1; A.swz = tuning().warp_swz != 0 ? 1 : 0;
+    A.frames = frames;
     A.u1[0] = u1[0]; A.u1[1] = u1[1]; A.u2[0] = u2[0]; A.u2[1] = u2[1];
     A.I1w = I1w; A.I1wx = I1wx; A.I1wy = I1wy; A.grad = grad; A.rho = rho;
     A.tab = cubic_tab_dev;
     A.g = g;
     const CtlK ck = make_ctlk(ctl);
     const bool cpu = semantics == MI_SEM_CPU_REF;
+    if (frames) {
+        MI_REQUIRE(!(lds < 0 ? tuning().warp_lds != 0 : lds != 0) && warp_tile() == 32 && tuning().warp_np == 2, MI_ERR_BAD_ARG,
+                   "frames in place: the gathering warp of 32 x 2 patches, two per wave, only");
+        const dim3 grid(div_up(g.w, 32 * 2), div_up(g.h, 4 * 2), g.batch);
+        if (cpu && fast) hipLaunchKernelGGL((k_warp6<MI_SEM_CPU_REF, 32, 2, true, true>), grid, dim3(256), 0, s, A, ck, cur_host);
+        else if (cpu) hipLaunchKernelGGL((k_warp6<MI_SEM_CPU_REF, 32, 2, false, true>), grid, dim3(256), 0, s, A, ck, cur_host);
+        else if (fast) hipLaunchKernelGGL((k_warp6<MI_SEM_CUDA_COMPAT, 32, 2, true, true>), grid, dim3(256), 0, s, A, ck, cur_host);
+        else hipLaunchKernelGGL((k_warp6<MI_SEM_CUDA_COMPAT, 32, 2, false, true>), grid, dim3(256), 0, s, A, ck, cur_host);
+        MI_HIP_TRY(hipGetLastError());
+        return MI_OK;
+    }
     if (lds < 0 ? tuning().warp_lds != 0 : lds != 0) {
 #ifndef MIFLOW_EXPERIMENTS
         set_error("the LDS-staged warp (k_warp_lds) exists in the experiments build only (-DMIFLOW_EXPERIMENTS)");
diff --git a/opencv_contrib_amd/csrc/tvl1_warp_px.h b/opencv_contrib_amd/csrc/tvl1_warp_px.h
--- a/opencv_contrib_amd/csrc/tvl1_warp_px.h
+++ b/opencv_contrib_amd/csrc/tvl1_warp_px.h
@@ -7,6 +7,19 @@
 
 typedef float f4u __attribute__((ext_vector_type(4), aligned(4)));
 typedef float f2u __attribute__((ext_vector_type(2), aligned(4)));
+
+constexpr float kFrameScale = 255.0f;
+template <bool INPL, class V>
+__device__ __forceinline__ V frame_load(const float *q)
+{
+    if constexpr (INPL) {
+        typedef const __attribute__((address_space(1))) char *gcchar_ptr;
+        typedef const __attribute__((address_space(1))) V *gv_ptr;
+        return *reinterpret_cast<gv_ptr>((gcchar_ptr) reinterpret_cast<const char *>(q));
+    } else {
+        return *reinterpret_cast<const V *>(q);
+    }
+}
 
 __device__ __forceinline__ float bicubic_coeff_cuda6(float x_)
 {
@@ -80,10 +93,14 @@
     }
 }
 
+template <bool INPL = false>
 __device__ __forceinline__ void fetch3b(__amdgpu_buffer_rsrc_t rs, int W, int H, int ld, int cx, int cy, float &v, float &vx, float &vy)
 {
     const unsigned ro = (unsigned)cy * (unsigned)ld;
-    const auto L = [&](unsigned e) { return __uint_as_float(__builtin_amdgcn_raw_buffer_load_b32(rs, 4u * e, 0, 0)); };
+    const auto L = [&](unsigned e) {
+        const float t = __uint_as_float(__builtin_amdgcn_raw_buffer_load_b32(rs, 4u * e, 0, 0));
+        return INPL ? t * kFrameScale : t;
+    };
     v = L(ro + cx);
     vx = 0.5f * (L(ro + min(cx + 1, W - 1)) - L(ro + max(cx - 1, 0)));
     vy = 0.5f * (L((unsigned)min(cy + 1, H - 1) * (unsigned)ld + cx) - L((unsigned)max(cy - 1, 0) * (unsigned)ld + cx));
@@ -116,33 +133,49 @@
 {
     return (unsigned)(sx - 1) < (unsigned)max(W - 5, 0) && (unsigned)(sy - 1) < (unsigned)max(H - 5, 0);
 }
+template <bool INPL = false>
 __device__ __forceinline__ void window_gather(float (&R)[6][6], const float *P, int ld, int sx, int sy)
 {
     const float *q = P + (long long)(sy - 1) * ld + (sx - 1);
     {
-        const f4u a = *reinterpret_cast<const f4u *>(q + 1);
+        const f4u a = frame_load<INPL, f4u>(q + 1);
         R[0][1] = a.x; R[0][2] = a.y; R[0][3] = a.z; R[0][4] = a.w;
     }
 #pragma unroll
     for (int r = 1; r < 5; ++r) {
         const float *qr = q + (long long)r * ld;
-        const f4u a = *reinterpret_cast<const f4u *>(qr);
-        const f2u c = *reinterpret_cast<const f2u *>(qr + 4);
+        const f4u a = frame_load<INPL, f4u>(qr);
+        const f2u c = frame_load<INPL, f2u>(qr + 4);
         R[r][0] = a.x; R[r][1] = a.y; R[r][2] = a.z; R[r][3] = a.w; R[r][4] = c.x; R[r][5] = c.y;
     }
     {
-        const f4u a = *reinterpret_cast<const f4u *>(q + (long long)5 * ld + 1);
+        const f4u a = frame_load<INPL, f4u>(q + (long long)5 * ld + 1);
         R[5][1] = a.x; R[5][2] = a.y; R[5][3] = a.z; R[5][4] = a.w;
     }
-}
-
-template <int SEM>
+    if constexpr (INPL) {
+#pragma unroll
+        for (int r = 0; r < 6; ++r)
+#pragma unroll
+            for (int c = 0; c < 6; ++c)
+                if (!((r == 0 || r == 5) && (c == 0 || c == 5))) R[r][c] = R[r][c] * kFrameScale;
+    }
+}
+
+template <bool INPL>
+__device__ __forceinline__ unsigned frame_extent_bytes(int W, int H, int ld)
+{
+    return INPL ? ((unsigned)(H - 1) * (unsigned)ld + (unsigned)W) * 4u : (unsigned)H * (unsigned)ld * 4u;
+}
+template <int SEM, bool INPL = false>
 __device__ __forceinline__ void window_border(const float *P, int W, int H, int ld, int sx, int sy, const float (&wxv)[4], const float (&wyv)[4],
                                               float &v0, float &v1, float &v2)
 {
     if (SEM == MI_SEM_CPU_REF) {
-        const __amdgpu_buffer_rsrc_t rs = __builtin_amdgcn_make_buffer_rsrc(const_cast<float *>(P), 0, (unsigned)H * (unsigned)ld * 4u, 0x00020000);
-        const auto L = [&](unsigned e) { return __uint_as_float(__builtin_amdgcn_raw_buffer_load_b32(rs, 4u * e, 0, 0)); };
+        const __amdgpu_buffer_rsrc_t rs = __builtin_amdgcn_make_buffer_rsrc(const_cast<float *>(P), 0, frame_extent_bytes<INPL>(W, H, ld), 0x00020000);
+        const auto L = [&](unsigned e) {
+            const float v = __uint_as_float(__builtin_amdgcn_raw_buffer_load_b32(rs, 4u * e, 0, 0));
+            return INPL ? v * kFrameScale : v;
+        };
         unsigned cxs[6];
 #pragma unroll
         for (int c = 0; c < 6; ++c) cxs[c] = (unsigned)min(max(sx - 1 + c, 0), W - 1);
@@ -181,7 +214,7 @@
         }
         v0 = win4 ? s0 : b0; v1 = win4 ? s1 : b1; v2 = win4 ? s2 : b2;
     } else {
-        const __amdgpu_buffer_rsrc_t rs = __builtin_amdgcn_make_buffer_rsrc(const_cast<float *>(P), 0, (unsigned)H * (unsigned)ld * 4u, 0x00020000);
+        const __amdgpu_buffer_rsrc_t rs = __builtin_amdgcn_make_buffer_rsrc(const_cast<float *>(P), 0, frame_extent_bytes<INPL>(W, H, ld), 0x00020000);
         float sum = 0.f, sumx = 0.f, sumy = 0.f, wsum = 0.f;
 #pragma unroll 1
         for (int j = 0; j < 4; ++j) {
@@ -189,7 +222,7 @@
             const float wyj = j == 0 ? wyv[0] : j == 1 ? wyv[1] : j == 2 ? wyv[2] : wyv[3];
             float t0[4], t1[4], t2[4];
 #pragma unroll
-            for (int i = 0; i < 4; ++i) fetch3b(rs, W, H, ld, min(max(sx + i, 0), W - 1), min(max(cy, 0), H - 1), t0[i], t1[i], t2[i]);
+            for (int i = 0; i < 4; ++i) fetch3b<INPL>(rs, W, H, ld, min(max(sx + i, 0), W - 1), min(max(cy, 0), H - 1), t0[i], t1[i], t2[i]);
 #pragma unroll
             for (int i = 0; i < 4; ++i) {
                 const float wgt = wxv[i] * wyj;
@@ -204,11 +237,11 @@
     }
 }
 
-template <int SEM, bool FAST>
-__device__ __forceinline__ void warp_px(const Warp6Args &A, const float *s_tab, const float *P, int x, int y, long long o, float u1v,
+template <int SEM, bool FAST, bool INPL = false>
+__device__ __forceinline__ void warp_px(const Warp6Args &A, const float *s_tab, const float *P, int ld, int x, int y, long long o, float u1v,
                                         float u2v, float i0)
 {
-    const int W = A.g.w, H = A.g.h, ld = A.g.ld;
+    const int W = A.g.w, H = A.g.h;
     int sx, sy;
     float wxv[4], wyv[4];
     warp_coords<SEM>(s_tab, x, y, u1v, u2v, sx, sy, wxv, wyv);
@@ -216,10 +249,10 @@
     float v0, v1, v2;
     if (window_interior(sx, sy, W, H)) {
         float R[6][6];
-        window_gather(R, P, ld, sx, sy);
+        window_gather<INPL>(R, P, ld, sx, sy);
         window_sums<SEM, FAST>(R, wxv, wyv, v0, v1, v2);
     } else {
-        window_border<SEM>(P, W, H, ld, sx, sy, wxv, wyv, v0, v1, v2);
+        window_border<SEM, INPL>(P, W, H, ld, sx, sy, wxv, wyv, v0, v1, v2);
     }
     if (A.I1w) A.I1w[o] = v0;
     A.I1wx[o] = v1;
```
